# refresh-bio/kmer-db

Hardware: AMD Instinct MI355X
Metric: all2all k-mer pair-comparisons/sec (higher is better)
Workload: dtype u32

## Files before the change

kmer-db_amd/csrc/a2a_blocks.hip:

```cpp
#include "device_common.h"
#include "engine_internal.h"

#include "prim.h"

#include <algorithm>
#include <chrono>
#include <cmath>
#include <cstdio>
#include <cstdlib>
#include <cstring>

enum : uint32_t {
    KCTR_CHUNKS = 0,
    KCTR_POOL_OVERFLOW,
    KCTR_PAIR_OVERFLOW,
    KCTR_NWIDE,
    KCTR_LIST_OVERFLOW,
    KCTR_RAW = 5,
    KCTR_RECORDS = 6,
    KCTR_RECORDS_HI = 7,
    KCTR_SLOW = 8,
    KCTR_WIDE_OVERFLOW = 9,
    KCTR_WIDE_RECORDS = 10,
    KCTR_ROWJOBS = 11,
// ... 97 lines not shown
    A.t_slot = lds; A.t_key = lds + (1u << tbits); A.tmask = (1u << tbits) - 1u;
    A.sub = wave_id % KMDB_SUBPOOLS; A.wsub = A.sub; A.stock = 0; A.next = 0; A.wstock = 0; A.wnext = 0; A.dslot = 0; A.dopen = 0;
    if (tbits == 0) return;
    for (uint32_t e = lane; e <= A.tmask; e += WAVE) { A.t_slot[e] = KEY_NONE; if (!A.direct) A.t_key[e] = KEY_NONE; }
    lds_sync();
}
template <class PV> __device__ __forceinline__ uint32_t arena_take(WaveArena& A, const PV& pv, uint32_t s, uint32_t lane) {
    if (A.stock == 0) {
        uint32_t base = 0;
        A.sub = (A.sub + 61u) % KMDB_SUBPOOLS;
        if (lane == 0) base = atomicAdd(&pool_cold(pv)->sub_cursor[A.sub * 16u], ARENA_GRAB);
        base = bcast(base, 0);
        if (base + ARENA_GRAB > pool_cold(pv)->sub_cap) {
            if (lane == 0) atomicOr(&pool_cold(pv)->counters[KCTR_POOL_OVERFLOW], 1u);
            base = pool_cold(pv)->sub_cap - ARENA_GRAB;
        }
        A.next = base; A.stock = ARENA_GRAB;
    }
    const uint32_t id = A.next * KMDB_SUBPOOLS + A.sub;
    ++A.next; --A.stock;
    if (lane == 0) pool_cold(pv)->chunk_key[id] = s;
    return id;
}
template <class PV> __device__ __forceinline__ uint32_t arena_take_wide(WaveArena& A, const PV& pv, uint32_t lane) {
    if (A.wstock == 0) {
        uint32_t base = 0;
        A.wsub = (A.wsub + 61u) % KMDB_SUBPOOLS;
        if (lane == 0) base = atomicAdd(&pool_cold(pv)->wsub_cursor[A.wsub * 16u], WIDE_GRAB);
        base = bcast(base, 0);
        if (base + WIDE_GRAB > pool_cold(pv)->wsub_cap) {
            if (lane == 0) atomicOr(&pool_cold(pv)->counters[KCTR_WIDE_OVERFLOW], 1u);
            base = pool_cold(pv)->wsub_cap - WIDE_GRAB;
        }
        A.wnext = base; A.wstock = WIDE_GRAB;
    }
    const uint32_t id = A.wnext * KMDB_SUBPOOLS + A.wsub;
    ++A.wnext; --A.wstock;
    return id;
}
template <class PV> __device__ __forceinline__ Resv arena_reserve_wide(WaveArena& A, const PV& pv, uint32_t cnt, uint32_t lane) {
    if (!A.dopen) { A.dslot = arena_take_wide(A, pv, lane) << WCH_SHIFT; A.dopen = 1; }
    const uint32_t v = A.dslot, rem = WCH_REC - (v & (WCH_REC - 1u));
    if (cnt < rem) { A.dslot = v + cnt; return Resv{v, cnt, 0u}; }
    if (cnt == rem) { A.dopen = 0; return Resv{v, cnt, 0u}; }
    const uint32_t nv = arena_take_wide(A, pv, lane) << WCH_SHIFT;
    A.dslot = nv + (cnt - rem);
    return Resv{v, rem, nv};
}
__device__ __forceinline__ Resv arena_reserve(WaveArena& A, const PoolView& pv, uint32_t ent, uint32_t s, uint32_t cnt, uint32_t lane) {
    const uint32_t e = ent & A.tmask;
    uint32_t v = A.t_slot[e];
    if (A.direct) {
        if (v == KEY_NONE) v = arena_take(A, pv, s, lane) << CH_SHIFT;
    } else {
        const uint32_t key = A.t_key[e];
        if (key != s) {
            if (key != KEY_NONE && lane == 0) pv.chunk_fill[v >> CH_SHIFT] = v & (CH_REC - 1u);
            v = arena_take(A, pv, s, lane) << CH_SHIFT;
        }
    }
    const uint32_t rem = CH_REC - (v & (CH_REC - 1u));
    Resv r{v, cnt, 0u};
    uint32_t nkey = s, nv = v + cnt;
    if (cnt >= rem) {
        if (lane == 0) pv.chunk_fill[v >> CH_SHIFT] = CH_REC;
        if (cnt == rem) { nkey = KEY_NONE; nv = KEY_NONE; }
        else {
            nv = arena_take(A, pv, s, lane) << CH_SHIFT;
            r = Resv{v, rem, nv};
            nv += cnt - rem;
        }
    }
    if (lane == 0) { A.t_slot[e] = nv; if (!A.direct) A.t_key[e] = nkey; }
    lds_sync();
    return r;
}
template <class PV> __device__ __forceinline__ void arena_finish(const WaveArena& A, const PV& pv, uint32_t lane) {
    if (A.tmask == 0) return;
    for (uint32_t e = lane; e <= A.tmask; e += WAVE) {
        const uint32_t v = A.t_slot[e];
        if (v != KEY_NONE && (A.direct || A.t_key[e] != KEY_NONE)) pool_cold(pv)->chunk_fill[v >> CH_SHIFT] = v & (CH_REC - 1u);
    }
}

template <class PV> __device__ __forceinline__ void wide_emit(WaveArena& A, const PV& pv, bool on, unsigned long long rows, unsigned long long cols, uint32_t w, uint32_t stream,
                                          uint32_t lane, unsigned long long lt_mask) {
    const uint32_t dbits = pv.pshift ? (64u - pv.pshift - 2u < 16u ? 64u - pv.pshift - 2u : 16u) : pv.dbits;
    const uint32_t dmask = (1u << dbits) - 1u;
    uint32_t j = 0;
    for (;;) {
        const unsigned long long grp = __ballot(on);
        if (!grp) break;
        const Resv r = arena_reserve_wide(A, pv, (uint32_t)__popcll(grp), lane);
        if (on) {
            const uint32_t slot = resv_slot(r, (uint32_t)__popcll(grp & lt_mask));
            if (pv.pshift) {
                pv.wrec[slot] = WideRec{rows, cols | ((unsigned long long)((w & dmask) | (j << dbits)) << pv.pshift)};
                pv.wkey[slot] = stream;
            } else {
                pv.wrec[slot] = WideRec{rows, cols};
                pv.wkey[slot] = stream | (((w & dmask) | (j << dbits)) << pv.kbits);
            }
        }
        w >>= dbits; ++j;
        on = on && w != 0;
    }
}
__device__ __forceinline__ uint32_t wide_weight(uint32_t key, uint32_t kbits, uint32_t dbits) {
    const uint32_t f = key >> kbits, dig = f & ((1u << dbits) - 1u), j = f >> dbits;
    const uint32_t sh = j * dbits;
    return sh < 32u ? dig << sh : 0u;
}
struct RowTab { uint32_t* pos; uint32_t* end; uint32_t n; };
__host__ __device__ inline size_t rowtab_bytes(uint32_t n_rows) { return ((size_t)8 * n_rows + 15) & ~(size_t)15; }
__device__ __forceinline__ void rowtab_init(RowTab& R, uint32_t* lds, uint32_t n, uint32_t lane) {
    R.pos = lds; R.end = lds + n; R.n = n;
    for (uint32_t e = lane; e < 2u * n; e += WAVE) lds[e] = 0u;
    lds_sync();
}
template <class PV> __device__ __forceinline__ void row_emit(WaveArena& A, const PV& pv, const RowTab& R, bool on, uint32_t X, unsigned long long rows, unsigned long long cols,
                                         uint32_t w, uint32_t stream, uint32_t lane, unsigned long long lt_mask) {
    const uint32_t dbits = pv.pshift ? (64u - pv.pshift - 2u < 16u ? 64u - pv.pshift - 2u : 16u) : pv.dbits;
    const uint32_t dmask = (1u << dbits) - 1u;
    uint32_t j = 0;
    for (;;) {
        const unsigned long long onm = __ballot(on);
        if (!onm) break;
        const uint32_t pX = (uint32_t)__shfl_up((int)X, 1, WAVE);
        const bool lead = on && (lane == 0u || !((onm >> (lane - 1u)) & 1ull) || pX != X);
        const unsigned long long leaders = __ballot(lead);
        uint32_t ll = lane, cnt = 0;
        if (on) {
            ll = 63u - (uint32_t)__builtin_clzll(leaders & (lt_mask | (1ull << lane)));
            const unsigned long long above = ll == 63u ? 0ull : ~((2ull << ll) - 1ull);
            const unsigned long long after = (leaders | ~onm) & above;
            cnt = (after ? (uint32_t)__builtin_ctzll(after) : 64u) - ll;
        }
        uint32_t old = 0, end = 0;
        if (lead) { end = R.end[X]; old = atomicAdd(&R.pos[X], cnt); }
        uint32_t p = (uint32_t)__shfl((int)old, (int)ll, WAVE) + (lane - ll);
        const uint32_t e = (uint32_t)__shfl((int)end, (int)ll, WAVE);
        bool ovf = on && p >= e;
        unsigned long long pend = __ballot(ovf);
        while (pend) {
            const uint32_t l0 = (uint32_t)__builtin_ctzll(pend);
            const uint32_t X0 = bcast(X, l0), e0 = bcast(e, l0);
            lds_sync();
            const uint32_t tot = R.pos[X0];
            const uint32_t over = tot - e0;
            const uint32_t nnew = (over + CH_REC - 1u) >> CH_SHIFT;
            if (lane == 0 && e0) pool_cold(pv)->chunk_fill[(e0 - 1u) >> CH_SHIFT] = CH_REC;
            const bool mine = ovf && X == X0;
            const uint32_t qv = p - e0;
            uint32_t cl = 0;
            for (uint32_t i = 0; i < nnew; ++i) {
                cl = arena_take(A, pv, pool_cold(pv)->n_states + X0, lane);
                if (lane == 0 && i + 1u < nnew) pool_cold(pv)->chunk_fill[cl] = CH_REC;
                if (mine && (qv >> CH_SHIFT) == i) p = (cl << CH_SHIFT) | (qv & (CH_REC - 1u));
            }
            if (lane == 0) { R.pos[X0] = (cl << CH_SHIFT) + (over - ((nnew - 1u) << CH_SHIFT)); R.end[X0] = (cl << CH_SHIFT) + CH_REC; }
            lds_sync();
            ovf = ovf && !mine;
            pend = __ballot(ovf);
        }
        if (on) {
            if (pv.pshift) {
                ((WideRec*)pv.rec)[p] = WideRec{rows, cols | ((unsigned long long)((w & dmask) | (j << dbits)) << pv.pshift)};
                pv.recw[p] = stream;
            } else {
                ((WideRec*)pv.rec)[p] = WideRec{rows, cols};
                pv.recw[p] = stream | (((w & dmask) | (j << dbits)) << pv.kbits);
            }
        }
        w >>= dbits; ++j;
        on = on && w != 0;
    }
}
template <class PV> __device__ __forceinline__ void rowtab_finish(const RowTab& R, const PV& pv, uint32_t lane) {
    lds_sync();
    for (uint32_t X = lane; X < R.n; X += WAVE) {
        const uint32_t e = R.end[X];
        if (e) pool_cold(pv)->chunk_fill[(e - 1u) >> CH_SHIFT] = CH_REC - (e - R.pos[X]);
    }
}
template <bool ROWS, class PV>
__device__ __forceinline__ void rec_emit(WaveArena& A, const PV& pv, const RowTab& R, bool on, uint32_t X, unsigned long long rows, unsigned long long cols,
                                         uint32_t w, uint32_t stream, uint32_t lane, unsigned long long lt_mask) {
    if constexpr (ROWS) row_emit(A, pv, R, on, X, rows, cols, w, stream, lane, lt_mask);
    else wide_emit(A, pv, on, rows, cols, w, stream, lane, lt_mask);
}
__device__ __forceinline__ void rec_store_diag(const PoolView& pv, uint32_t slot, unsigned long long rows, uint32_t w) {
    const uint32_t ch = slot >> CH_SHIFT, r = slot & (CH_REC - 1u);
    ((unsigned long long*)(pv.rec + ((size_t)ch << (CH_SHIFT + 4))))[r] = rows;
    pv.recw[slot] = w;
}

__global__ void fill_u32_kernel(uint32_t* __restrict__ p, uint32_t n, uint32_t v) {
    const uint32_t i = blockIdx.x * blockDim.x + threadIdx.x;
    if (i < n) p[i] = v;
}
__global__ void iota_u32_kernel(uint32_t* __restrict__ p, uint32_t n) {
    const uint32_t i = blockIdx.x * blockDim.x + threadIdx.x;
    if (i < n) p[i] = i;
}

struct K0Params {
    const uint2* k0in;
    const uint32_t* bitrel;
    const uint64_t* blkbase;
    const uint64_t* bits;
    const uint32_t* perm;
    uint32_t P;
    uint32_t short_ids;
    BlockMap bm;
    unsigned long long* p0_mask;
    uint32_t* p0_info;
    uint32_t* pair_ofs;
    uint16_t* pair_blk;
    unsigned long long* pair_mask;
    uint32_t* pair_cursor;
    uint32_t n_regions, region_cap, spill_cap;
    uint32_t* counters;
};

constexpr int K0_RELW = 8;
constexpr int K0_SINGLE_PASS = 1;
template <bool LONG>
__global__ __launch_bounds__(256) void k0_decode_kernel(const K0Params q) {
    const uint32_t t = blockIdx.x * blockDim.x + threadIdx.x;
    const uint32_t lane = threadIdx.x & 63u;
    uint32_t i = 0;
    bool live;
    if (q.perm) {
        live = t < q.P;
        if (live) i = q.perm[t];
    } else {
        __shared__ uint32_t bins[64];
        __shared__ uint16_t order[256];
        if (threadIdx.x < 64) bins[threadIdx.x] = 0;
        __syncthreads();
        const uint2 kt = t < q.P ? q.k0in[t] : make_uint2(0u, 0u);
        const uint32_t tl = kmdb_k0_l(kt), tbits = kmdb_k0_bits(kt);
        uint32_t key = 0;
        if (t < q.P && tl > 1 && !kmdb_long_node(tl, tbits, q.short_ids)) {
            key = 1u + (tbits - (tl - 1u));
            key = key > 63u ? 63u : key;
        }
        atomicAdd(&bins[63u - key], 1u);
        __syncthreads();
        if (threadIdx.x < 64) {
            const uint32_t c = bins[threadIdx.x];
            bins[threadIdx.x] = wave_incl_scan(c, threadIdx.x) - c;
        }
        __syncthreads();
        order[atomicAdd(&bins[63u - key], 1u)] = (uint16_t)threadIdx.x;
        __syncthreads();
        i = blockIdx.x * blockDim.x + order[threadIdx.x];
        live = i < q.P;
    }
    const BlockMap bm = q.bm;
    const uint2 km = live ? q.k0in[i] : make_uint2(0u, 0u);
    const uint32_t l = kmdb_k0_l(km), last = kmdb_k0_last(km), nbits = kmdb_k0_bits(km);
    if (!q.perm && kmdb_long_node(l, nbits, q.short_ids)) live = false;
    using Cursor = RunCursor32<LONG ? 16 : 6, LONG>;
    uint32_t npairs = 0, blk0 = 0, need = 0, span = 0, bit0 = 0;
    unsigned long long mask0 = 0, m1 = 0, m2 = 0;
    bool second_pass = false, from_words = false;
    uint64_t pos = 0;
    unsigned long long rel_w[K0_RELW];
    uint32_t rel_i[K0_RELW], rel_n = 0;
#pragma unroll
    for (int e = 0; e < K0_RELW; ++e) { rel_w[e] = 0; rel_i[e] = 0; }
    auto rel_push = [&](uint32_t idx, unsigned long long w) {
#pragma unroll
        for (int e = 0; e < K0_RELW; ++e) if (rel_n == (uint32_t)e) { rel_w[e] = w; rel_i[e] = idx; }
        ++rel_n;
    };
    auto rel_blocks = [&](bool write, uint32_t id0, uint32_t o) -> uint32_t {
        const unsigned long long wm = bm.width == 64 ? ~0ull : (1ull << bm.width) - 1ull;
        uint32_t curblk = 0xFFFFFFFFu, cnt = 0;
        unsigned long long cacc = 0;
        auto flushb = [&]() {
// ... 152 lines not shown
__device__ __forceinline__ TrConst tr_const(uint32_t lane) {
    TrConst c;
    const uint32_t m[5] = {0x0000FFFFu, 0x00FF00FFu, 0x0F0F0F0Fu, 0x33333333u, 0x55555555u};
#pragma unroll
    for (int k = 0; k < 5; ++k) {
        const uint32_t s = 16u >> k;
        const bool up = (lane & s) != 0;
        c.amt[k] = up ? s : 32u - s;
        c.msk[k] = up ? m[k] : ~m[k];
    }
    return c;
}
__device__ __forceinline__ uint32_t tr_fetch(uint32_t v, int k, bool up16) {
    if (k == 0) {
        const auto a = __builtin_amdgcn_permlane16_swap(v, v, false, false);
        return up16 ? a[0] : a[1];
    }
    if (k == 1) return (uint32_t)__builtin_amdgcn_update_dpp((int)v, (int)v, 0x128, 0xF, 0xF, false);
    if (k == 2) {
        const int a = __builtin_amdgcn_update_dpp((int)v, (int)v, 0x104, 0xF, 0x5, false);
        return (uint32_t)__builtin_amdgcn_update_dpp(a, (int)v, 0x114, 0xF, 0xA, false);
    }
    if (k == 3) return (uint32_t)__builtin_amdgcn_update_dpp((int)v, (int)v, 0x4E, 0xF, 0xF, false);
    return (uint32_t)__builtin_amdgcn_update_dpp((int)v, (int)v, 0xB1, 0xF, 0xF, false);
}
__device__ __forceinline__ unsigned long long transpose64(unsigned long long x, const TrConst& c) {
    uint32_t lo = (uint32_t)x, hi = (uint32_t)(x >> 32);
    {
        const auto r = __builtin_amdgcn_permlane32_swap(lo, hi, false, false);
        lo = r[0]; hi = r[1];
    }
    const bool up16 = c.msk[0] == 0x0000FFFFu;
#pragma unroll
    for (int k = 0; k < 5; ++k) {
        const uint32_t pl = tr_fetch(lo, k, up16), ph = tr_fetch(hi, k, up16);
        const uint32_t rl = __builtin_amdgcn_alignbit(pl, pl, c.amt[k]), rh = __builtin_amdgcn_alignbit(ph, ph, c.amt[k]);
        asm("v_bfi_b32 %0, %1, %2, %0" : "+v"(lo) : "v"(c.msk[k]), "v"(rl));
        asm("v_bfi_b32 %0, %1, %2, %0" : "+v"(hi) : "v"(c.msk[k]), "v"(rh));
    }
    return ((unsigned long long)hi << 32) | lo;
}

typedef int k2_v4i __attribute__((ext_vector_type(4)));
typedef int k2_v16i __attribute__((ext_vector_type(16)));

constexpr uint32_t BNONE = 0x7FFFu;
struct NSum { unsigned long long m0, m1; uint32_t bw; };

__device__ __forceinline__ NSum nsum_make(uint32_t b0, unsigned long long m0, uint32_t b1, unsigned long long m1, bool wide) {
    return NSum{m0, m1, b0 | (b1 << 15) | ((wide ? 1u : 0u) << 30)};
}
__device__ __forceinline__ NSum nsum_merge(const NSum& T, const NSum& S) {
    const uint32_t Tb0 = T.bw & 0x7FFFu, Tb1 = (T.bw >> 15) & 0x7FFFu, Sb0 = S.bw & 0x7FFFu, Sb1 = (S.bw >> 15) & 0x7FFFu;
    bool wide = (((T.bw | S.bw) >> 30) & 1u) != 0;
    if (Tb0 == BNONE) return S;
    if (Sb0 == BNONE) return T;
    if (Sb0 == Tb0) return nsum_make(Sb0, S.m0 | T.m0, Sb1, S.m1, wide || Tb1 != BNONE);
    if (Tb1 == BNONE) return nsum_make(Tb0, T.m0, Sb0, S.m0, wide || Sb1 != BNONE);
    if (Tb1 == Sb0) return nsum_make(Tb0, T.m0, Sb0, T.m1 | S.m0, wide || Sb1 != BNONE);
    return nsum_make(Tb0, T.m0, Tb1, T.m1, true);
}
__device__ __forceinline__ NSum nsum_shfl(const NSum& s, int src) {
    return NSum{shfl64(s.m0, src), shfl64(s.m1, src), (uint32_t)__shfl((int)s.bw, src, WAVE)};
}
__device__ __forceinline__ NSum nsum_shfl_up(const NSum& s, int d) {
    return NSum{shfl_up64(s.m0, d), shfl_up64(s.m1, d), (uint32_t)__shfl_up((int)s.bw, d, WAVE)};
}

struct NParams {
    const uint32_t* nl;
    const int32_t* parent;
    const uint32_t* w;
    const uint16_t* dflag;
    const uint32_t* seg_anc;
    const uint32_t* seg_anc_n;
    const unsigned long long* p0_mask;
    const uint32_t* p0_info;
    const uint32_t* pair_ofs;
    const uint16_t* pair_blk;
    const unsigned long long* pair_mask;
    ulonglong2* fn_mask;
    uint32_t* fn_blk;
    unsigned long long* widebits;
    uint32_t P, nseg_nodes, n_segs, chain_cap;
    uint32_t emit_lo, emit_hi;
    uint32_t tbits, n_keys;
    uint32_t all_wide;
    PoolView pool;
    uint32_t* M;
    uint32_t N, bwidth;
    unsigned char* touched;
    uint32_t* direct_ctr;
    unsigned long long* dmask;
    uint32_t* dwx;
    uint32_t* slice_cnt;
    uint32_t dbg;
};
constexpr int K1N_WAVES = 4;
__host__ __device__ inline size_t k1n_wave_bytes(uint32_t chain_cap, uint32_t tbits, uint32_t n_states, uint32_t n_rows) {
    return (((size_t)chain_cap * 20 + 15) & ~(size_t)15) + arena_table_bytes(tbits, n_states) + rowtab_bytes(n_rows);
}

template <int MODE, int MINW, bool ROWS>
__global__ __launch_bounds__(WAVE * K1N_WAVES) __attribute__((amdgpu_waves_per_eu(MINW, 8))) void k1n_kernel(const NParams q) {
    constexpr bool DIRECT = MODE == 1, FLAT = MODE == 2;
    extern __shared__ __attribute__((aligned(16))) unsigned char lds_raw[];
    __shared__ unsigned long long lut_ff[DIRECT ? 256 : 1], lut_01[DIRECT ? 256 : 1];
    __shared__ __attribute__((aligned(16))) unsigned char wbuf[DIRECT ? K1N_WAVES : 1][64];
    const uint32_t lane = lane_id();
    const uint32_t wave = threadIdx.x >> 6;
    const uint32_t seg = blockIdx.x * (blockDim.x >> 6) + wave;
    if (DIRECT) {
        for (uint32_t b = threadIdx.x; b < 256u; b += blockDim.x) {
            unsigned long long v = 0;
#pragma unroll
            for (int i = 0; i < 8; ++i) v |= ((b >> i) & 1u) ? 0xFFull << (8 * i) : 0ull;
            lut_ff[b] = v;
            lut_01[b] = v & 0x0101010101010101ull;
        }
        __syncthreads();
    }
    if (seg >= q.n_segs) return;
    const uint32_t n_rows = ROWS ? q.n_keys : 0u;
    unsigned char* wbase = lds_raw + k1n_wave_bytes(q.chain_cap, q.tbits, q.n_keys, n_rows) * wave;
    uint32_t* table = (uint32_t*)wbase;
    ulonglong2* chain_m = (ulonglong2*)(wbase + arena_table_bytes(q.tbits, q.n_keys));
    uint32_t* chain_b = (uint32_t*)(chain_m + q.chain_cap);
    const unsigned long long lt_mask = (1ull << lane) - 1ull;
    RowTab RT{nullptr, nullptr, 0u};
    if constexpr (ROWS) rowtab_init(RT, (uint32_t*)(wbase + (((size_t)q.chain_cap * 20 + 15) & ~(size_t)15) + arena_table_bytes(q.tbits, q.n_keys)), n_rows, lane);
    PoolRef pv{};
    pv.k = &((KARG(NParams))__builtin_amdgcn_kernarg_segment_ptr())->pool;
    pv.kbits = q.pool.kbits; pv.dbits = q.pool.dbits; pv.pshift = q.pool.pshift;
    if constexpr (ROWS) { pv.rec = q.pool.rec; pv.recw = q.pool.recw; } else { pv.wkey = q.pool.wkey; pv.wrec = q.pool.wrec; }
    const uint32_t first = seg * q.nseg_nodes;
    const uint32_t end = (q.P - first) < q.nseg_nodes ? q.P : first + q.nseg_nodes;

    auto locals = [&](uint32_t info, unsigned long long m0, uint32_t e1blk, unsigned long long e1mask) -> NSum {
        const uint32_t np = info >> 16;
        if (np == 0) return nsum_make(BNONE, 0ull, BNONE, 0ull, false);
        if (np == 1) return nsum_make(info & 0xFFFFu, m0, BNONE, 0ull, false);
        return nsum_make(info & 0xFFFFu, m0, e1blk, e1mask, np > 2);
    };

    {
        KARG(NParams) qr = kernarg_reread<NParams>();
        const uint32_t d = qr->seg_anc_n[seg];
        NSum carry = nsum_make(BNONE, 0ull, BNONE, 0ull, false);
        for (uint32_t cb = 0; cb < d; cb += WAVE) {
            const uint32_t k = cb + lane;
            const bool on = k < d;
            NSum S = nsum_make(BNONE, 0ull, BNONE, 0ull, false);
            if (on) {
                const uint32_t node = qr->seg_anc[(size_t)seg * q.chain_cap + k];
                const uint32_t info = q.p0_info[node];
                uint32_t e1b = BNONE; unsigned long long e1m = 0;
                if ((info >> 16) > 1u) { const uint32_t po = q.pair_ofs[node]; e1b = q.pair_blk[po]; e1m = q.pair_mask[po]; }
                S = locals(info, q.p0_mask[node], e1b, e1m);
            }
            if (lane == 0) S = nsum_merge(carry, S);
#pragma unroll
            for (int s = 1; s < WAVE; s <<= 1) {
                const NSum o = nsum_shfl_up(S, s);
                if (lane >= (uint32_t)s) S = nsum_merge(o, S);
            }
            if (on) { chain_m[k] = make_ulonglong2(S.m0, S.m1); chain_b[k] = S.bw; }
            carry = nsum_shfl(S, WAVE - 1);
        }
        lds_sync();
    }

    uint32_t nx_nl = 0, nx_w = 0, nx_info = 0, nx_df = 0, nx_e1b = BNONE, nx_po = 0;
    int32_t nx_par = -1;
    unsigned long long nx_m0 = 0, nx_e1m = 0;
    uint32_t n2_nl = 0, n2_w = 0, n2_info = 0, n2_df = 0x7FFFu, n2_po = 0;
    int32_t n2_par = -1;
    unsigned long long n2_m0 = 0;
    auto fetch2 = [&](uint32_t b0) {
        const uint32_t ii = b0 + lane;
        const bool v = ii < end;
        n2_nl = v ? q.nl[ii] : 0u;
        n2_w = v ? q.w[ii] : 0u;
        n2_par = v ? q.parent[ii] : -1;
        n2_df = v ? q.dflag[ii] : 0x7FFFu;
        n2_info = v ? q.p0_info[ii] : 0u;
        n2_m0 = v ? q.p0_mask[ii] : 0ull;
        n2_po = v ? q.pair_ofs[ii] : 0u;
    };
    auto advance = [&]() {
        nx_nl = n2_nl; nx_w = n2_w; nx_par = n2_par; nx_df = n2_df; nx_info = n2_info; nx_m0 = n2_m0; nx_po = n2_po;
        nx_e1b = BNONE; nx_e1m = 0;
        if ((nx_info >> 16) > 1u) { nx_e1b = q.pair_blk[nx_po]; nx_e1m = q.pair_mask[nx_po]; }
    };
    fetch2(first); advance();
    if (first + WAVE < end) fetch2(first + WAVE); else { n2_nl = 0; n2_w = 0; n2_par = -1; n2_df = 0x7FFFu; n2_info = 0; n2_m0 = 0; n2_po = 0; }
    WaveArena A;
    arena_init(A, table, MODE != 0 ? 0u : q.tbits, q.n_keys, seg, lane);
    k2_v16i c00 = {}, c10 = {}, c11 = {};
    uint32_t curX = BNONE, n_direct = 0;
    uint32_t flat_n = 0;
    auto dflush = [&]() {
        const uint32_t half = lane >> 5, l31 = lane & 31u;
        const uint32_t rb = curX * q.bwidth;
        uint32_t* const Mb = q.M + (tri64((uint64_t)rb) + rb);
        const uint32_t lim = q.N - rb;
#pragma unroll
        for (int r = 0; r < 16; ++r) {
            const uint32_t row0 = (uint32_t)((r & 3) + 8 * (r >> 2)) + 4u * half, row1 = row0 + 32u;
            const uint32_t o0 = rb * row0 + row0 * (row0 - 1u) / 2u + l31, o1 = rb * row1 + row1 * (row1 - 1u) / 2u + l31;
            const uint32_t v00 = (uint32_t)c00[r], v10 = (uint32_t)c10[r], v11 = (uint32_t)c11[r];
            if (v00 && l31 < row0 && row0 < lim) atomicAdd(Mb + o0, v00);
            if (v10 && row1 < lim) atomicAdd(Mb + o1, v10);
            if (v11 && l31 < row0 && row1 < lim) atomicAdd(Mb + o1 + 32u, v11);
            c00[r] = 0; c10[r] = 0; c11[r] = 0;
        }
        if (lane == 0 && q.touched) q.touched[tri32(curX) + curX] = 1;
    };
    for (uint32_t base = first; base < end; base += WAVE) {
        const uint32_t idx = base + lane;
        const bool valid = idx < end;
        const uint32_t nl = nx_nl, w = nx_w, info = nx_info, df = nx_df, e1b = nx_e1b;
        const int32_t par = nx_par;
        const unsigned long long m0 = nx_m0, e1m = nx_e1m;
        if (base + WAVE < end) {
            advance();
            if (base + 2 * WAVE < end) fetch2(base + 2 * WAVE); else { n2_nl = 0; n2_w = 0; n2_par = -1; n2_df = 0x7FFFu; n2_info = 0; n2_m0 = 0; n2_po = 0; }
        }
        const uint32_t dep = df & 0x7FFFu;
        NSum S = locals(info, m0, e1b, e1m);
        if (valid && par >= 0 && par < (int32_t)base) {
            const ulonglong2 cm = chain_m[dep - 2u];
            S = nsum_merge(NSum{cm.x, cm.y, chain_b[dep - 2u]}, S);
        }
        int pl = (valid && par >= (int32_t)base) ? (int)(par - (int32_t)base) : -1;
        while (__ballot(pl >= 0)) {
            const int src = pl >= 0 ? pl : (int)lane;
            const NSum o = nsum_shfl(S, src);
            if (pl >= 0) S = nsum_merge(o, S);
            const int npl = __shfl(pl, src, WAVE);
            pl = pl >= 0 ? npl : -1;
        }
        const bool wide = valid && ((S.bw >> 30) & 1u);
        const uint32_t w0 = S.bw & 0x7FFFu, w1 = (S.bw >> 15) & 0x7FFFu;
        const unsigned long long F0 = S.m0, F1 = w1 != BNONE ? S.m1 : 0ull;
        {
            const unsigned long long wb = __ballot(wide);
            if (lane == 0) q.widebits[base >> 6] = wb;
        }
        if (__ballot(wide)) {
            const int pl0 = (valid && par >= (int32_t)base) ? (int)(par - (int32_t)base) : (int)lane;
            NSum Pp = nsum_shfl(S, pl0);
            if (valid && par >= 0 && par < (int32_t)base) { const ulonglong2 cm = chain_m[dep - 2u]; Pp = NSum{cm.x, cm.y, chain_b[dep - 2u]}; }
            if (wide && par >= 0 && !((Pp.bw >> 30) & 1u)) {
                const uint32_t pb0 = Pp.bw & 0x7FFFu, pb1 = (Pp.bw >> 15) & 0x7FFFu;
                q.fn_mask[idx] = make_ulonglong2(Pp.m0, pb1 != BNONE ? Pp.m1 : 0ull);
                q.fn_blk[idx] = (pb0 == BNONE ? 0xFFFFu : pb0) | ((pb1 == BNONE ? 0xFFFFu : pb1) << 16);
            }
        }
        const bool act = valid && !wide && w != 0 && nl >= 2u && w0 != BNONE && idx >= q.emit_lo && idx < q.emit_hi;
        auto first_block_records = [&]() {
            bool d0 = act && __popcll(F0) >= 2;
            if (FLAT) {
                const bool dd = d0 && w < 128u;
                const unsigned long long bm = __ballot(dd);
                if (dd) {
                    const uint32_t slot = first + flat_n + (uint32_t)__popcll(bm & lt_mask);
                    q.dmask[slot] = F0; q.dwx[slot] = w | (w0 << 8);
                }
                flat_n += (uint32_t)__popcll(bm);
                d0 = d0 && !dd;
            }
            if (DIRECT) {
                const bool dd = d0 && w < 128u;
                const unsigned long long pend = __ballot(dd);
                if (pend) {
                    if (curX == BNONE) curX = bcast(w0, (uint32_t)__builtin_ctzll(pend));
                    const bool mine = dd && w0 == curX;
                    n_direct += (uint32_t)__popcll(__ballot(mine));
                    if (!(q.dbg & 2u)) {
                    const TrConst trc = tr_const(lane);
                    const unsigned long long Rt = transpose64(mine ? F0 : 0ull, trc);
                    unsigned long long ra0, ra1;
                    {
                        const auto a = __builtin_amdgcn_permlane32_swap((uint32_t)Rt, (uint32_t)Rt, false, false);
                        const auto b = __builtin_amdgcn_permlane32_swap((uint32_t)(Rt >> 32), (uint32_t)(Rt >> 32), false, false);
                        ra0 = ((unsigned long long)b[0] << 32) | a[0];
                        ra1 = ((unsigned long long)b[1] << 32) | a[1];
                    }
                    wbuf[wave][lane] = (unsigned char)(mine ? w : 0u);
                    lds_sync();
                    const uint32_t half = lane >> 5;
                    auto spread = [&](unsigned long long word, uint32_t shift, const unsigned long long* lut) -> k2_v4i {
                        const uint32_t f = (uint32_t)(word >> shift) & 0xFFFFu;
                        k2_v4i r;
                        const unsigned long long lo = lut[f & 0xFFu], hi = lut[f >> 8];
                        r[0] = (int)(uint32_t)lo; r[1] = (int)(uint32_t)(lo >> 32); r[2] = (int)(uint32_t)hi; r[3] = (int)(uint32_t)(hi >> 32);
                        return r;
                    };
    #pragma unroll 1
                    for (uint32_t kh = 0; kh < 2; ++kh) {
                        const uint32_t shift = 32u * kh + 16u * half;
                        k2_v4i a0 = spread(ra0, shift, lut_ff), a1 = spread(ra1, shift, lut_ff);
                        const k2_v4i b0 = spread(ra0, shift, lut_01), b1 = spread(ra1, shift, lut_01);
                        const k2_v4i wv = *(const k2_v4i*)(wbuf[wave] + shift);
                        a0 &= wv; a1 &= wv;
                        c00 = __builtin_amdgcn_mfma_i32_32x32x32_i8(a0, b0, c00, 0, 0, 0);
                        c10 = __builtin_amdgcn_mfma_i32_32x32x32_i8(a1, b0, c10, 0, 0, 0);
                        c11 = __builtin_amdgcn_mfma_i32_32x32x32_i8(a1, b1, c11, 0, 0, 0);
                    }
                    lds_sync();
                    }
                    d0 = d0 && !mine;
                }
            }
            if (MODE == 0 && !q.all_wide) {
                unsigned long long pend = __ballot(d0);
                while (pend) {
                    const uint32_t X0 = bcast(w0, (uint32_t)__builtin_ctzll(pend));
                    const bool mine = d0 && w0 == X0;
                    const unsigned long long bc = __ballot(mine);
                    const Resv r = arena_reserve(A, q.pool, X0, tri32(X0) + X0, (uint32_t)__popcll(bc), lane);
                    if (mine) rec_store_diag(q.pool, resv_slot(r, (uint32_t)__popcll(bc & lt_mask)), F0, w);
                    pend &= ~bc;
                }
            } else {
                rec_emit<ROWS>(A, pv, RT, d0, w0, F0, F0, w, tri32(w0) + w0, lane, lt_mask);
            }
        };
        if (!DIRECT) first_block_records();
        {
            const bool act2 = act && F1 != 0;
            if (__ballot(act2)) {
                rec_emit<ROWS>(A, pv, RT, act2, w1, F1, F0, w, tri32(w1) + w0, lane, lt_mask);
                rec_emit<ROWS>(A, pv, RT, act2 && __popcll(F1) >= 2, w1, F1, F1, w, tri32(w1) + w1, lane, lt_mask);
            }
        }
        if (base + WAVE < end) {
            uint32_t m = dep;
#pragma unroll
            for (int s = 1; s < WAVE; s <<= 1) {
                const uint32_t o = (uint32_t)__shfl_down((int)m, s, WAVE);
                if (lane + (uint32_t)s < (uint32_t)WAVE) m = o < m ? o : m;
            }
            uint32_t later = (uint32_t)__shfl_down((int)m, 1, WAVE);
            if (lane == (uint32_t)WAVE - 1u) later = 0xFFFFFFFFu;
            if (valid && dep < later) { chain_m[dep - 1u] = make_ulonglong2(S.m0, S.m1); chain_b[dep - 1u] = S.bw; }
            lds_sync();
        }
        if (DIRECT) first_block_records();
    }
    if (DIRECT && curX != BNONE && !(q.dbg & 1u)) dflush();
    KARG(NParams) qe = kernarg_reread<NParams>();
    if (DIRECT && lane == 0 && n_direct) atomicAdd(&qe->direct_ctr[(seg % KMDB_SUBPOOLS) * 16u], n_direct);
    if (FLAT && lane == 0) { qe->slice_cnt[seg] = flat_n; if (flat_n) atomicAdd(&qe->direct_ctr[(seg % KMDB_SUBPOOLS) * 16u], flat_n); }
    if constexpr (MODE == 0) arena_finish(A, q.pool, lane);
    if constexpr (ROWS) rowtab_finish(RT, pv, lane);
}

constexpr uint32_t K2D_SLICES = 2;
struct DParams {
    const unsigned long long* dmask;
    const uint32_t* dwx;
    const uint32_t* slice_cnt;
    uint32_t n_segs, nseg_nodes, slices;
    uint32_t* M;
    uint32_t N, bwidth;
    unsigned char* touched;
};
__global__ __launch_bounds__(256) __attribute__((amdgpu_waves_per_eu(4, 8))) void k2d_kernel(const DParams q) {
    __shared__ unsigned long long lut_ff[256], lut_01[256];
    __shared__ __attribute__((aligned(16))) unsigned char wbuf[4][64];
    {
        unsigned long long v = 0;
#pragma unroll
        for (int i = 0; i < 8; ++i) v |= ((threadIdx.x >> i) & 1u) ? 0xFFull << (8 * i) : 0ull;
        lut_ff[threadIdx.x] = v;
        lut_01[threadIdx.x] = v & 0x0101010101010101ull;
        __syncthreads();
    }
    const uint32_t lane = threadIdx.x & 63u, wave = threadIdx.x >> 6;
    const uint32_t half = lane >> 5, l31 = lane & 31u;
    const uint32_t s0 = (blockIdx.x * 4u + wave) * q.slices;
    if (s0 >= q.n_segs) return;
    const uint32_t s1 = s0 + q.slices < q.n_segs ? s0 + q.slices : q.n_segs;
    const TrConst trc = tr_const(lane);
    auto spread = [&](unsigned long long word, uint32_t shift, const unsigned long long* lut) -> k2_v4i {
        const uint32_t f = (uint32_t)(word >> shift) & 0xFFFFu;
        k2_v4i r;
        const unsigned long long lo = lut[f & 0xFFu], hi = lut[f >> 8];
        r[0] = (int)(uint32_t)lo; r[1] = (int)(uint32_t)(lo >> 32); r[2] = (int)(uint32_t)hi; r[3] = (int)(uint32_t)(hi >> 32);
        return r;
    };
    uint32_t s = s0, n = q.slice_cnt[s0], b = 0;
    auto skip_empty = [&]() { while (b >= n && s + 1u < s1) { ++s; n = q.slice_cnt[s]; b = 0; } };
    skip_empty();
    unsigned long long nm = 0; uint32_t nwx = 0;
    auto fetch = [&]() {
        nm = 0; nwx = 0;
        if (b + lane < n) { const size_t i = (size_t)s * q.nseg_nodes + b + lane; nm = q.dmask[i]; nwx = q.dwx[i]; }
    };
    if (b < n) fetch();
    unsigned long long m = 0, pend = 0;
    uint32_t wx = 0;
    auto next_step = [&]() -> bool {
        if (b >= n) return false;
        m = nm; wx = nwx;
        b += WAVE;
        skip_empty();
        if (b < n) fetch();
        pend = __ballot(m != 0ull);
        return true;
    };
    for (;;) {
        while (!pend && next_step()) {}
        if (!pend) break;
        const uint32_t X0 = bcast(wx >> 8, (uint32_t)__builtin_ctzll(pend));
        k2_v16i c00 = {}, c10 = {}, c11 = {};
        for (;;) {
            const bool mine = ((pend >> lane) & 1ull) && (wx >> 8) == X0;
            const unsigned long long bm = __ballot(mine);
            if (!bm) break;
            pend &= ~bm;
            const unsigned long long Rt = transpose64(mine ? m : 0ull, trc);
            unsigned long long ra0, ra1;
            {
                const auto a = __builtin_amdgcn_permlane32_swap((uint32_t)Rt, (uint32_t)Rt, false, false);
                const auto c = __builtin_amdgcn_permlane32_swap((uint32_t)(Rt >> 32), (uint32_t)(Rt >> 32), false, false);
                ra0 = ((unsigned long long)c[0] << 32) | a[0];
                ra1 = ((unsigned long long)c[1] << 32) | a[1];
            }
            wbuf[wave][lane] = (unsigned char)(mine ? (wx & 0xFFu) : 0u);
            lds_sync();
#pragma unroll 1
            for (uint32_t kh = 0; kh < 2; ++kh) {
                const uint32_t shift = 32u * kh + 16u * half;
                k2_v4i a0 = spread(ra0, shift, lut_ff), a1 = spread(ra1, shift, lut_ff);
                const k2_v4i b0 = spread(ra0, shift, lut_01), b1 = spread(ra1, shift, lut_01);
                const k2_v4i wv = *(const k2_v4i*)(wbuf[wave] + shift);
                a0 &= wv; a1 &= wv;
                c00 = __builtin_amdgcn_mfma_i32_32x32x32_i8(a0, b0, c00, 0, 0, 0);
                c10 = __builtin_amdgcn_mfma_i32_32x32x32_i8(a1, b0, c10, 0, 0, 0);
                c11 = __builtin_amdgcn_mfma_i32_32x32x32_i8(a1, b1, c11, 0, 0, 0);
            }
            lds_sync();
            if (pend || !next_step()) break;
        }
        const uint32_t rb = X0 * q.bwidth;
        uint32_t* const Mb = q.M + (tri64((uint64_t)rb) + rb);
        const uint32_t lim = q.N - rb;
        uint32_t h4 = 4u * half, lc = l31;
        asm volatile("" : "+v"(h4), "+v"(lc));
#pragma unroll
        for (int r = 0; r < 16; ++r) {
            const uint32_t row0 = (uint32_t)((r & 3) + 8 * (r >> 2)) + h4, row1 = row0 + 32u;
            const uint32_t o0 = rb * row0 + row0 * (row0 - 1u) / 2u + lc, o1 = rb * row1 + row1 * (row1 - 1u) / 2u + lc;
            const uint32_t v00 = (uint32_t)c00[r], v10 = (uint32_t)c10[r], v11 = (uint32_t)c11[r];
            if (v00 && lc < row0 && row0 < lim) atomicAdd(Mb + o0, v00);
            if (v10 && row1 < lim) atomicAdd(Mb + o1, v10);
            if (v11 && lc < row0 && row1 < lim) atomicAdd(Mb + o1 + 32u, v11);
        }
        if (lane == 0 && q.touched) q.touched[tri32(X0) + X0] = 1;
    }
}

__global__ void wide_count_kernel(const unsigned long long* __restrict__ bits, uint32_t n_words, uint32_t* __restrict__ cnt) {
    const uint32_t i = blockIdx.x * blockDim.x + threadIdx.x;
    if (i < n_words) cnt[i] = (uint32_t)__popcll(bits[i]);
    else if (i == n_words) cnt[i] = 0;
}
__global__ void wide_expand_kernel(const unsigned long long* __restrict__ bits, const uint32_t* __restrict__ base, uint32_t n_words,
                                   uint32_t* __restrict__ widx, uint32_t cap, uint32_t* __restrict__ counters) {
    const uint32_t i = blockIdx.x * blockDim.x + threadIdx.x;
    if (i == 0) counters[KCTR_NWIDE] = base[n_words];
    if (i >= n_words) return;
    unsigned long long b = bits[i];
    uint32_t o = base[i];
    while (b) {
        const uint32_t k = (uint32_t)__builtin_ctzll(b);
        b &= b - 1;
        if (o < cap) widx[o] = i * 64u + k;
        ++o;
    }
}

constexpr uint32_t BLK_NONE = 0xFFFFu;
struct LSum { unsigned long long lm; uint32_t c, fb, lb; };
__device__ __forceinline__ LSum lsum_none() { return LSum{0ull, 0u, BLK_NONE, BLK_NONE}; }
__device__ __forceinline__ LSum lsum_merge(const LSum& A, const LSum& B) {
    if (B.c == 0u) return A;
    if (A.c == 0u) return B;
    const bool seam = A.lb == B.fb;
    return LSum{(B.c == 1u && seam) ? (A.lm | B.lm) : B.lm, A.c + B.c - (seam ? 1u : 0u), A.fb, B.lb};
}
__device__ __forceinline__ LSum lsum_shfl(const LSum& s, int src) {
    return LSum{shfl64(s.lm, src), (uint32_t)__shfl((int)s.c, src, WAVE), (uint32_t)__shfl((int)s.fb, src, WAVE), (uint32_t)__shfl((int)s.lb, src, WAVE)};
}
__device__ __forceinline__ LSum lsum_shfl_up(const LSum& s, int d) {
    return LSum{shfl_up64(s.lm, d), (uint32_t)__shfl_up((int)s.c, d, WAVE), (uint32_t)__shfl_up((int)s.fb, d, WAVE), (uint32_t)__shfl_up((int)s.lb, d, WAVE)};
}
__device__ __forceinline__ LSum lsum_of_fn(uint32_t fb, const ulonglong2& fm) {
    const uint32_t b0 = fb & 0xFFFFu, b1 = fb >> 16;
    if (b0 == BLK_NONE) return lsum_none();
    if (b1 == BLK_NONE) return LSum{fm.x, 1u, b0, b0};
    return LSum{fm.y, 2u, b0, b1};
}

struct L2View {
    uint32_t on, min_blocks;
    uint32_t node_cap, W;
    uint32_t ent_cap;
    uint32_t* cursors;
    unsigned long long* bitmap;
    uint32_t* ent_g;
    uint16_t* ent_blk;
    unsigned long long* ent_mask;
    uint32_t* node_w;
};
struct WParams {
    const uint32_t* widx;
    uint32_t n_wide;
    const uint32_t* nl;
    const int32_t* parent;
    const uint32_t* w;
    const uint16_t* dflag;
    const unsigned long long* widebits;
    const uint32_t* wide_base;
    const unsigned long long* p0_mask;
    const uint32_t* p0_info;
    const uint32_t* pair_ofs;
    const uint16_t* pair_blk;
    const unsigned long long* pair_mask;
    const ulonglong2* fn_mask;
    const uint32_t* fn_blk;
    const uint32_t* seg_anc;
    const uint32_t* seg_anc_n;
    uint32_t run_nodes;
    uint32_t n_runs, n_waves;
    uint32_t* run_ctr;
    uint32_t chain_cap, arena_cap, e_cap;
    uint32_t n_rows;
    uint32_t emit_lo, emit_hi;
    PoolView pool;
    L2View l2;
};
constexpr int K1W_WAVES = 2;
constexpr int K1W_MINW_FEW = 5;

constexpr uint32_t L2_MIN_BLOCKS = 24;
constexpr uint32_t L2_NODE_GRAB = 16, L2_ENT_GRAB = 1024, L2_SUB = 16;
constexpr uint32_t K1W_QCAP = 64;
constexpr uint32_t K1W_HEAVY = 11;
constexpr uint32_t K1W_OXCAP = 96;
constexpr uint32_t K1W_CTRS = 16;
constexpr uint32_t K1W_ARENA_MIN = 256;
enum : uint32_t { WB_NONE = 0, WB_FN = 1, WB_LANE = 2, WB_CHAIN = 3 };
struct K1WLds {
    unsigned long long* ent_mask;
    unsigned long long* e_mask;
    unsigned long long* ch_last;
    unsigned long long* own_m0;
    unsigned long long* own_desc;
    uint32_t* ch_node;
    unsigned long long* ox_mask;
    uint32_t* own_po;
// ... 290 lines not shown
            const uint32_t slen = len - pre;
            L.own_m0[lane] = m0; L.own_po[lane] = po;
            {
                const uint32_t nx = np > 1u ? np - 1u : 0u;
                const uint32_t xincl = wave_incl_scan(nx, lane);
                const uint32_t x0 = xincl - nx;
                const bool fits = nx && xincl <= K1W_OXCAP;
                if (fits) for (uint32_t t = 0; t < nx; ++t) { L.ox_blk[x0 + t] = qb->pair_blk[po + t]; L.ox_mask[x0 + t] = qb->pair_mask[po + t]; }
                L.own_desc[lane] = (unsigned long long)(b0 & 0xFFFFu) | ((unsigned long long)(link & 0xFFFFu) << 16) | ((unsigned long long)(fits ? x0 : 0xFFFFu) << 32) |
                                   ((unsigned long long)(np & 0x3FFFu) << 48) | ((unsigned long long)base << 62);
            }
            lds_sync();
            const bool need = valid && (act || lane == nv - 1u);
            uint32_t fin = 0, last_start = 0;
            while (fin < nv) {
                const uint32_t c = (lane >= fin && need) ? slen : 0u;
                const uint32_t incl = wave_incl_scan(c, lane);
                const unsigned long long over = __ballot(incl > qb->arena_cap);
                uint32_t hi = over ? (uint32_t)__builtin_ctzll(over) : (uint32_t)WAVE;
                if (hi <= fin) { if (lane == 0) atomicOr(&pool_cold(pv)->counters[KCTR_LIST_OVERFLOW], 1u); hi = fin + 1u; }
                const bool on = need && lane >= fin && lane < hi && incl <= qb->arena_cap;
                const uint32_t start = incl - c;
                if (on) {
                    uint32_t pos = start + slen, cur = 0xFFFFFFFFu;
                    unsigned long long curm = 0;
                    auto rflush = [&]() { if (cur != 0xFFFFFFFFu) { --pos; L.ent_blk[pos] = (uint16_t)cur; L.ent_mask[pos] = curm; } };
                    auto rpush = [&](uint32_t blk, unsigned long long mask) {
                        if (blk == cur) curm |= mask;
                        else { rflush(); cur = blk; curm = mask; }
                    };
                    uint32_t y = lane;
                    for (;;) {
                        const unsigned long long dsc = L.own_desc[y];
                        const unsigned long long ym0 = L.own_m0[y];
                        const uint32_t ynp = (uint32_t)(dsc >> 48) & 0x3FFFu, yb = (uint32_t)(dsc >> 62), ylink = (uint32_t)(dsc >> 16) & 0xFFFFu;
                        if (ynp > 1u) {
                            const uint32_t yox = (uint32_t)(dsc >> 32) & 0xFFFFu;
                            const uint32_t ynx = ynp - 1u;
                            if (yox != 0xFFFFu) for (uint32_t t = ynx; t-- > 0u;) rpush(L.ox_blk[yox + t], L.ox_mask[yox + t]);
                            else {
                                const uint32_t ypo = L.own_po[y];
                                KARG(WParams) qp = kernarg_reread<WParams>();
                                for (uint32_t t = ynx; t-- > 0u;) rpush(qp->pair_blk[ypo + t], qp->pair_mask[ypo + t]);
                            }
                        }
                        if (ynp) rpush((uint32_t)dsc & 0xFFFFu, ym0);
                        if (yb == WB_LANE) { y = ylink; continue; }
                        if (yb == WB_FN) {
                            if ((tfnb >> 16) != BLK_NONE) rpush(tfnb >> 16, tfny);
                            if ((tfnb & 0xFFFFu) != BLK_NONE) rpush(tfnb & 0xFFFFu, tfnx);
                        } else if (yb == WB_CHAIN) {
                            const uint32_t cs = ylink;
                            const uint32_t cl = L.ch_len[cs];
                            if (cl) rpush(L.e_blk[cl - 1u], L.ch_last[cs]);
                        }
                        break;
                    }
                    rflush();
                }
                L.st_start[lane] = (uint16_t)start; L.st_pre[lane] = (uint16_t)pre;
                if (lane == nv - 1u && on) last_start = start;
                lds_sync();
                emit(on && act, len, wv);
                fin = hi;
            }
            {
                uint32_t mdep = dep;
#pragma unroll
                for (int sft = 1; sft < WAVE; sft <<= 1) {
                    const uint32_t o = (uint32_t)__shfl_down((int)mdep, sft, WAVE);
                    if (lane + (uint32_t)sft < (uint32_t)WAVE) mdep = o < mdep ? o : mdep;
                }
                uint32_t later = (uint32_t)__shfl_down((int)mdep, 1, WAVE);
                if (lane == (uint32_t)WAVE - 1u) later = 0xFFFFFFFFu;
                if (valid && dep < later && dep - 1u < qb->chain_cap) { L.ch_node[dep - 1u] = node; L.ch_len[dep - 1u] = (uint16_t)len; L.ch_last[dep - 1u] = S.lm; }
                const uint32_t ll = bcast(slen, nv - 1u), ls = bcast(last_start, nv - 1u), lp = bcast(pre, nv - 1u);
                for (uint32_t e = lane; e < ll; e += WAVE) { L.e_blk[lp + e] = L.ent_blk[ls + e]; L.e_mask[lp + e] = L.ent_mask[ls + e]; }
                lds_sync();
            }
        }
    }
    arena_finish(A, pv, lane);
    if constexpr (ROWS) rowtab_finish(RT, pv, lane);
    if (lane == 0 && n_miss) atomicAdd(&pool_cold(pv)->counters[KCTR_SLOW], n_miss);
    if constexpr (L2) if (lane == 0 && l2_nodes) atomicAdd(&pool_cold(pv)->counters[KCTR_L2_NODES], l2_nodes);
}

struct K2Item {
    uint32_t X, Y, count;
    const uint32_t* ids;
    const uint32_t* fills;
    const WideRec* srec;
    const uint32_t* skey;
    uint32_t kbits, dbits;
    uint32_t pshift;
    uint32_t rect_cols;
    uint32_t n_rec;
    const unsigned char* rec;
    const uint32_t* recw;
};
constexpr uint32_t CH_STEPS = CH_REC / 64u;
template <bool SORTED>
__device__ __forceinline__ void k2_fetch(const K2Item& it, bool diag, uint32_t st, uint32_t lane, bool weighted, unsigned long long& R,
                                         unsigned long long& Cc, uint32_t& W) {
    R = 0; Cc = 0; W = 0;
    if (st >= it.count) return;
    if (SORTED) {
        const uint32_t p = st * 64u + lane;
        if (p < it.n_rec) {
            const WideRec r = it.srec[p];
            R = r.rows; Cc = r.cols;
            if (it.pshift) {
                const uint32_t f = (uint32_t)(r.cols >> it.pshift), pd = 64u - it.pshift - 2u < 16u ? 64u - it.pshift - 2u : 16u;
                const uint32_t sh = (f >> pd) * pd;
                Cc = r.cols & ((1ull << it.pshift) - 1ull);
                W = sh < 32u ? (f & ((1u << pd) - 1u)) << sh : 0u;
            } else
            W = weighted ? wide_weight(it.skey[p], it.kbits, it.dbits) : 1u;
        }
    } else {
        const uint32_t ci = st / CH_STEPS, j = (st % CH_STEPS) * 64u + lane;
        if (j < it.fills[ci]) {
            const uint32_t id = it.ids[ci];
            const unsigned char* base = it.rec + ((size_t)id << (CH_SHIFT + 4));
            if (diag) { R = ((const unsigned long long*)base)[j]; Cc = R; }
            else { const ulonglong2 rc = ((const ulonglong2*)base)[j]; R = rc.x; Cc = rc.y; }
            W = weighted ? it.recw[((size_t)id << CH_SHIFT) + j] : 1u;
        }
    }
}


template <bool DIAG, bool SORTED>
__device__ __forceinline__ uint32_t k2_apply_mfma(const K2Item& it, uint32_t digit, uint32_t* acc,
                                                  unsigned char (*wbuf)[64], const unsigned long long* lut_ff, const unsigned long long* lut_01) {
    const uint32_t lane = threadIdx.x & 63u, wave = threadIdx.x >> 6;
    const uint32_t half = lane >> 5, l31 = lane & 31u;
    k2_v16i c00 = {}, c01 = {}, c10 = {}, c11 = {};
    auto spread = [&](unsigned long long word, uint32_t shift, const unsigned long long* lut) -> k2_v4i {
        const uint32_t f = (uint32_t)(word >> shift) & 0xFFFFu;
        k2_v4i r;
        const unsigned long long lo = lut[f & 0xFFu], hi = lut[f >> 8];
        r[0] = (int)(uint32_t)lo; r[1] = (int)(uint32_t)(lo >> 32); r[2] = (int)(uint32_t)hi; r[3] = (int)(uint32_t)(hi >> 32);
        return r;
    };
    unsigned long long nR = 0, nC = 0;
    uint32_t nW = 0, wor = 0;
    const TrConst trc = tr_const(lane);
    auto next_step = [&](uint32_t st) -> uint32_t {
        if (!SORTED) while (st < it.count && (st % CH_STEPS) * 64u >= it.fills[st / CH_STEPS]) st += 4;
        return st;
    };
    uint32_t cur = next_step(wave);
    k2_fetch<SORTED>(it, DIAG, cur, lane, true, nR, nC, nW);
    while (cur < it.count) {
        const unsigned long long R = nR, C = nC;
        const uint32_t W = nW;
        cur = next_step(cur + 4);
        k2_fetch<SORTED>(it, DIAG, cur, lane, true, nR, nC, nW);
        wor |= W;
        const unsigned long long Ct = transpose64(C, trc);
        const unsigned long long Rt = DIAG ? Ct : transpose64(R, trc);
        auto halves = [&](unsigned long long w, unsigned long long& w0, unsigned long long& w1) {
            const auto a = __builtin_amdgcn_permlane32_swap((uint32_t)w, (uint32_t)w, false, false);
            const auto b = __builtin_amdgcn_permlane32_swap((uint32_t)(w >> 32), (uint32_t)(w >> 32), false, false);
            w0 = ((unsigned long long)b[0] << 32) | a[0];
// ... 242 lines not shown
        }
        const uint32_t sh = 7u * digit;
#pragma unroll
        for (int r = 0; r < 16; ++r) {
            const uint32_t row0 = (uint32_t)((r & 3) + 8 * (r >> 2)) + 4u * half;
            const uint32_t v00 = (uint32_t)c00[r] << sh, v01 = (uint32_t)c01[r] << sh, v10 = (uint32_t)c10[r] << sh, v11 = (uint32_t)c11[r] << sh;
            if (v00 && (!diag || l31 < row0)) atomicAdd(&acc[row0 * 64 + l31], v00);
            if (v01 && (!diag || 32u + l31 < row0)) atomicAdd(&acc[row0 * 64 + 32u + l31], v01);
            if (v10 && (!diag || l31 < 32u + row0)) atomicAdd(&acc[(32u + row0) * 64 + l31], v10);
            if (v11 && (!diag || l31 < row0)) atomicAdd(&acc[(32u + row0) * 64 + 32u + l31], v11);
        }
#pragma unroll
        for (int d = 32; d >= 1; d >>= 1) wor |= (uint32_t)__shfl_xor((int)wor, d, WAVE);
        if (lane == 0 && wor) atomicOr(&wor_sh, wor);
        __syncthreads();
        if (digit == 4u || (wor_sh >> (7u * (digit + 1u))) == 0) break;
        __syncthreads();
    }
    if (threadIdx.x == 0 && touched) touched[t] = 1;
    for (uint32_t k = threadIdx.x; k < 64 * 64; k += 64 * L2_WAVES) {
        const uint32_t v = acc[k];
        if (!v) continue;
        const uint64_t row = (uint64_t)X * bwidth + (k >> 6), col = (uint64_t)Y * bwidth + (k & 63u);
        if (row < N && col < row) atomicAdd(&M[tri64(row) + col], v);
    }
}

constexpr uint32_t K2_WIN = 32;
constexpr int K2A_MIN_WAVES = 3;
__global__ __launch_bounds__(256) __attribute__((amdgpu_waves_per_eu(K2A_MIN_WAVES, 8))) void k2_apply_kernel(const unsigned char* __restrict__ rec, const uint32_t* __restrict__ recw,
                                                       const uint32_t* __restrict__ sorted_key, const uint32_t* __restrict__ sorted_id,
                                                       const uint32_t* __restrict__ chunk_fill, uint32_t n_states, const uint32_t* __restrict__ n_chunks_ptr,
                                                       uint32_t* __restrict__ M, uint32_t N, uint32_t bwidth, uint32_t win, unsigned char* __restrict__ touched) {
    __shared__ uint32_t acc[64 * 64];
    __shared__ __attribute__((aligned(16))) unsigned char wbuf[4][64];
    __shared__ unsigned long long lut_ff[256], lut_01[256];
    __shared__ uint32_t s_key[K2_WIN], s_id[K2_WIN], s_fill[K2_WIN];
    __shared__ uint32_t wor_sh;
    if (threadIdx.x < win) {
        const uint32_t j = blockIdx.x * win + threadIdx.x;
        const uint32_t key = j < *n_chunks_ptr ? sorted_key[j] : n_states;
        const uint32_t id = key < n_states ? sorted_id[j] : 0u;
        s_key[threadIdx.x] = key; s_id[threadIdx.x] = id; s_fill[threadIdx.x] = key < n_states ? chunk_fill[id] : 0u;
    }
    {
        unsigned long long v = 0;
#pragma unroll
        for (int i = 0; i < 8; ++i) v |= ((threadIdx.x >> i) & 1u) ? 0xFFull << (8 * i) : 0ull;
        lut_ff[threadIdx.x] = v;
        lut_01[threadIdx.x] = v & 0x0101010101010101ull;
    }
    __syncthreads();
    uint32_t a = 0;
    while (a < win && s_key[a] < n_states) {
        const uint32_t key = s_key[a];
        uint32_t b = a + 1;
        while (b < win && s_key[b] == key) ++b;
        K2Item it;
        {
            const uint32_t bucket = key;
            uint32_t X = (uint32_t)((__fsqrt_rn(8.0f * (float)bucket + 1.0f) - 1.0f) * 0.5f);
            while (tri32(X) > bucket) --X;
            while (tri32(X + 1u) <= bucket) ++X;
            it.X = X; it.Y = bucket - tri32(X);
            it.count = (b - a) * CH_STEPS; it.ids = s_id + a; it.fills = s_fill + a; it.srec = nullptr; it.n_rec = 0; it.rec = rec; it.recw = recw; it.rect_cols = 0; it.pshift = 0;
        }
        k2_run<false>(it, acc, &wor_sh, wbuf, lut_ff, lut_01, M, N, bwidth, touched);
        a = b;
    }
}

__global__ void count_chunks_kernel(const uint32_t* __restrict__ sorted_key, uint32_t pool_cap, uint32_t n_states, uint32_t* __restrict__ counters) {
    uint32_t lo = 0, hi = pool_cap;
    while (lo < hi) { const uint32_t mid = (lo + hi) >> 1; if (sorted_key[mid] < n_states) lo = mid + 1; else hi = mid; }
    counters[KCTR_CHUNKS] = lo;
}
__global__ void pool_used_kernel(const uint32_t* __restrict__ sub_cursor, const uint32_t* __restrict__ direct_ctr, uint32_t* __restrict__ counters) {
    uint32_t mx = 0, nd = 0;
    for (uint32_t p = threadIdx.x; p < KMDB_SUBPOOLS; p += 64u) { mx = max(mx, sub_cursor[p * 16u]); nd += direct_ctr[p * 16u]; }
#pragma unroll
    for (int d = 32; d >= 1; d >>= 1) { mx = max(mx, (uint32_t)__shfl_xor((int)mx, d, WAVE)); nd += (uint32_t)__shfl_xor((int)nd, d, WAVE); }
    if (threadIdx.x == 0) { counters[KCTR_POOL_USED] = mx * KMDB_SUBPOOLS; counters[KCTR_DIRECT] = nd; }
}
__global__ void count_raw_kernel(const uint32_t* __restrict__ wsub_cursor, uint32_t* __restrict__ counters) {
    uint32_t mx = 0;
    for (uint32_t p = 0; p < KMDB_SUBPOOLS; ++p) mx = max(mx, wsub_cursor[p * 16u]);
    counters[KCTR_RAW] = mx * KMDB_SUBPOOLS;
}

constexpr uint32_t CS_MAX_KEYS = 2048, CS_BLOCKS = 2048, CS_MAX_ROWS = 512;
constexpr uint32_t CS_BLOCKS_ONE = 3072;
__device__ __forceinline__ uint32_t stream_row(uint32_t s) {
    uint32_t X = (uint32_t)((__fsqrt_rn(8.0f * (float)s + 1.0f) - 1.0f) * 0.5f);
    while (tri32(X) > s) --X;
    while (tri32(X + 1u) <= s) ++X;
    return X;
}
struct CsRows {
    const uint32_t* row_start;
    const uint32_t* row_blk;
    const uint32_t* row_tab;
    uint32_t NB, chunk;
};
enum { CS_BY_STREAM = 0, CS_BY_ROW = 1, CS_IN_ROW = 2 };
struct CsJob { uint32_t lo, hi, n_bins, sub, tab, stride; };
__device__ __forceinline__ CsJob cs_job(int mode, uint32_t n, uint32_t n_keys, const CsRows& rows) {
    CsJob j{0u, 0u, n_keys, 0u, blockIdx.x, gridDim.x};
    if (mode != CS_IN_ROW) {
        const uint32_t vb = (gridDim.x & 7u) ? blockIdx.x : xcd_contiguous(blockIdx.x, gridDim.x);
        j.tab = vb;
        const uint32_t per_block = ((n + gridDim.x - 1u) / gridDim.x + 1023u) / 1024u * 1024u;
        const uint32_t lo = vb * per_block;
        if (lo < n) { j.lo = lo; j.hi = n - lo < per_block ? n : lo + per_block; }
        return j;
    }
    j.n_bins = 0;
    if (blockIdx.x >= rows.row_blk[rows.NB]) return j;
    uint32_t a = 0, b = rows.NB;
    while (b - a > 1u) { const uint32_t mid = (a + b) >> 1; if (rows.row_blk[mid] <= blockIdx.x) a = mid; else b = mid; }
    const uint32_t X = a, c = blockIdx.x - rows.row_blk[X];
    j.lo = rows.row_start[X] + c * rows.chunk;
    j.hi = rows.row_start[X + 1];
    if (j.hi - j.lo > rows.chunk) j.hi = j.lo + rows.chunk;
    j.n_bins = X + 1u; j.sub = tri32(X); j.tab = rows.row_tab[X] + c; j.stride = rows.row_blk[X + 1] - rows.row_blk[X];
    return j;
}
__device__ __forceinline__ uint32_t cs_bin(int mode, uint32_t key, uint32_t n_valid, uint32_t sub) {
    if (key >= n_valid) return 0xFFFFFFFFu;
    return mode == CS_BY_ROW ? stream_row(key) : key - sub;
}
__global__ void cs_rows_kernel(const uint32_t* __restrict__ O1, uint32_t NB, uint32_t chunk, uint32_t* __restrict__ row_start, uint32_t* __restrict__ row_blk,
                               uint32_t* __restrict__ row_tab) {
    for (uint32_t X = threadIdx.x; X <= NB; X += blockDim.x) row_start[X] = O1[(size_t)X * CS_BLOCKS];
    __syncthreads();
    if (threadIdx.x == 0) {
        uint32_t blk = 0, tab = 0;
        for (uint32_t X = 0; X < NB; ++X) {
            row_blk[X] = blk; row_tab[X] = tab;
            const uint32_t nch = (row_start[X + 1] - row_start[X] + chunk - 1u) / chunk;
            blk += nch; tab += nch * (X + 1u);
        }
        row_blk[NB] = blk; row_tab[NB] = tab;
    }
}
__global__ __launch_bounds__(256) void cs_hist_kernel(const uint32_t* __restrict__ wkey, uint32_t n, uint32_t n_valid, uint32_t n_keys, int mode, const CsRows rows,
                                                     uint32_t kmask, uint32_t* __restrict__ H) {
    extern __shared__ uint32_t cs_lds[];
    const CsJob job = cs_job(mode, n, n_keys, rows);
    for (uint32_t k = threadIdx.x; k < job.n_bins; k += blockDim.x) cs_lds[k] = 0;
    __syncthreads();
    for (uint32_t i0 = job.lo; i0 < job.hi; i0 += 8u * blockDim.x) {
        uint32_t kw[8];
#pragma unroll
        for (uint32_t j = 0; j < 8; ++j) {
            const uint32_t i = i0 + j * blockDim.x + threadIdx.x;
            kw[j] = i < job.hi ? wkey[i] : 0xFFFFFFFFu;
        }
#pragma unroll
        for (uint32_t j = 0; j < 8; ++j) {
            const uint32_t bin = kw[j] == 0xFFFFFFFFu ? 0xFFFFFFFFu : cs_bin(mode, kw[j] & kmask, n_valid, job.sub);
            if (bin < job.n_bins) atomicAdd(&cs_lds[bin], 1u);
        }
    }
    __syncthreads();
    for (uint32_t k = threadIdx.x; k < job.n_bins; k += blockDim.x) H[(size_t)job.tab + (size_t)k * job.stride] = cs_lds[k];
    if (mode != CS_IN_ROW && blockIdx.x == 0 && threadIdx.x == 0) H[(size_t)n_keys * gridDim.x] = 0;
}
constexpr uint32_t CS_TILE = 2048, CS_THREADS = 256;
__host__ __device__ inline size_t cs_scatter_lds(uint32_t n_keys, bool packed) { return (size_t)CS_TILE * (sizeof(WideRec) + (packed ? 4 : 8)) + (size_t)n_keys * 12 + CS_THREADS * 4 + 64; }
__global__ __launch_bounds__(CS_THREADS) void cs_scatter_kernel(const uint32_t* __restrict__ wkey, const WideRec* __restrict__ wrec, uint32_t n, uint32_t n_valid,
                                                         uint32_t n_keys, int mode, const CsRows rows, uint32_t kmask, const uint32_t* __restrict__ O,
                                                         uint32_t* __restrict__ swkey, WideRec* __restrict__ swrec, uint32_t packed) {
    extern __shared__ __attribute__((aligned(16))) unsigned char cs_raw[];
    WideRec* st_rec = (WideRec*)cs_raw;
    uint32_t* st_dst = (uint32_t*)(st_rec + CS_TILE);
    uint32_t* st_key = st_dst + CS_TILE;
    uint32_t* hist = st_key + (packed ? 0u : CS_TILE);
    uint32_t* toff = hist + n_keys;
    uint32_t* cursor = toff + n_keys;
    uint32_t* part = cursor + n_keys;
    const CsJob job = cs_job(mode, n, n_keys, rows);
    const uint32_t nb = job.n_bins, lo = job.lo, hi = job.hi;
    for (uint32_t k = threadIdx.x; k < nb; k += CS_THREADS) cursor[k] = O[(size_t)job.tab + (size_t)k * job.stride];
    constexpr uint32_t PER = CS_TILE / CS_THREADS;
    const uint32_t kper = (nb + CS_THREADS - 1u) / CS_THREADS;
    uint32_t nkw[PER];
    WideRec nrec[PER];
    auto fetch = [&](uint32_t t0) {
#pragma unroll
        for (uint32_t j = 0; j < PER; ++j) {
            const uint32_t i = t0 + j * CS_THREADS + threadIdx.x;
            nkw[j] = 0xFFFFFFFFu; nrec[j] = WideRec{0ull, 0ull};
            if (i < hi) { nkw[j] = wkey[i]; nrec[j] = wrec[i]; }
        }
    };
    if (lo < hi) fetch(lo);
    for (uint32_t t0 = lo; t0 < hi; t0 += CS_TILE) {
        for (uint32_t k = threadIdx.x; k < nb; k += CS_THREADS) hist[k] = 0;
        __syncthreads();
        uint32_t key[PER], kw[PER], rank[PER];
        WideRec rc[PER];
#pragma unroll
        for (uint32_t j = 0; j < PER; ++j) {
            kw[j] = nkw[j]; rc[j] = nrec[j];
            key[j] = cs_bin(mode, kw[j] & kmask, n_valid, job.sub);
            rank[j] = key[j] < nb ? atomicAdd(&hist[key[j]], 1u) : 0u;
        }
        if (t0 + CS_TILE < hi) fetch(t0 + CS_TILE);
        __syncthreads();
        uint32_t sum = 0;
        for (uint32_t k = threadIdx.x * kper; k < nb && k < (threadIdx.x + 1u) * kper; ++k) sum += hist[k];
        const uint32_t sincl = wave_incl_scan(sum, threadIdx.x & 63u);
        if ((threadIdx.x & 63u) == 63u) part[threadIdx.x >> 6] = sincl;
        __syncthreads();
        uint32_t run = sincl - sum;
        for (uint32_t k = 0; k < (threadIdx.x >> 6); ++k) run += part[k];
        const uint32_t tile_n = part[0] + part[1] + part[2] + part[3];
        for (uint32_t k = threadIdx.x * kper; k < nb && k < (threadIdx.x + 1u) * kper; ++k) { toff[k] = run; run += hist[k]; }
        __syncthreads();
#pragma unroll
        for (uint32_t j = 0; j < PER; ++j) {
            if (key[j] < nb) {
                const uint32_t p = toff[key[j]] + rank[j];
                st_rec[p] = rc[j];
                st_dst[p] = cursor[key[j]] + rank[j];
                if (!packed) st_key[p] = kw[j];
            }
        }
        __syncthreads();
        for (uint32_t k = threadIdx.x; k < nb; k += CS_THREADS) cursor[k] += hist[k];
        for (uint32_t p = threadIdx.x; p < tile_n; p += CS_THREADS) {
            const uint32_t d = st_dst[p];
            swrec[d] = st_rec[p];
            if (!packed) swkey[d] = st_key[p];
        }
        __syncthreads();
    }
}

constexpr uint32_t CT_THREADS = 1024, CT_SLOTS = 2048;
__device__ __forceinline__ void ct_group(uint32_t key, bool on, uint32_t* t_key, uint32_t* t_cnt, uint32_t& slot, uint32_t& rank) {
    for (uint32_t e = threadIdx.x; e < CT_SLOTS; e += CT_THREADS) { t_key[e] = 0xFFFFFFFFu; t_cnt[e] = 0u; }
    __syncthreads();
    slot = 0; rank = 0;
    if (on) {
        uint32_t h = (key * 2654435761u) >> 21;
        for (;;) {
            const uint32_t prev = atomicCAS(&t_key[h], 0xFFFFFFFFu, key);
            if (prev == 0xFFFFFFFFu || prev == key) break;
            h = (h + 1u) & (CT_SLOTS - 1u);
        }
        slot = h;
        rank = atomicAdd(&t_cnt[h], 1u);
    }
    __syncthreads();
}
__global__ __launch_bounds__(CT_THREADS) void ct_hist_kernel(const uint32_t* __restrict__ chunk_key, uint32_t n, uint32_t n_keys, uint32_t* __restrict__ hist) {
    __shared__ uint32_t t_key[CT_SLOTS], t_cnt[CT_SLOTS];
    const uint32_t i = blockIdx.x * CT_THREADS + threadIdx.x;
    const uint32_t k = i < n ? chunk_key[i] : 0xFFFFFFFFu;
    uint32_t slot, rank;
    ct_group(k, k < n_keys, t_key, t_cnt, slot, rank);
    for (uint32_t e = threadIdx.x; e < CT_SLOTS; e += CT_THREADS)
        if (t_cnt[e]) atomicAdd(&hist[t_key[e]], t_cnt[e]);
}
__global__ __launch_bounds__(CT_THREADS) void ct_scatter_kernel(const uint32_t* __restrict__ chunk_key, uint32_t n, uint32_t n_keys, uint32_t* __restrict__ cursor,
                                                               uint32_t* __restrict__ sorted_key, uint32_t* __restrict__ sorted_id) {
    __shared__ uint32_t t_key[CT_SLOTS], t_cnt[CT_SLOTS];
    const uint32_t i = blockIdx.x * CT_THREADS + threadIdx.x;
    const uint32_t k = i < n ? chunk_key[i] : 0xFFFFFFFFu;
    const bool on = k < n_keys;
    uint32_t slot, rank;
    ct_group(k, on, t_key, t_cnt, slot, rank);
    for (uint32_t e = threadIdx.x; e < CT_SLOTS; e += CT_THREADS)
        if (t_cnt[e]) t_cnt[e] = atomicAdd(&cursor[t_key[e]], t_cnt[e]);
    __syncthreads();
    if (on) {
        const uint32_t o = t_cnt[slot] + rank;
// ... 330 lines not shown
    int32_t y = on ? (int32_t)node : -1;
    while (y >= 0) {
        const uint2 km = q.k0in[y];
        const uint32_t l = kmdb_k0_l(km), last = kmdb_k0_last(km);
        if (l) {
            const uint64_t pos = q.blkbase[(uint32_t)y >> 8] + q.bitrel[y];
            uint32_t sum = 0;
            if (l > 1) { BitCursor c(q.bits, pos); for (uint32_t k = 0; k + 1 < l; ++k) sum += c.next(); }
            uint32_t id = last - sum;
            uint32_t fb[EST_NW], cb[EST_NW];
#pragma unroll
            for (int c = 0; c < EST_NW; ++c) { fb[c] = __umulhi(id, q.magics[c]); cb[c] = fb[c]; nblk[c] += 1; }
            if (l > 1) {
                BitCursor c2(q.bits, pos);
                for (uint32_t k = 0; k + 1 < l; ++k) {
                    id += c2.next();
#pragma unroll
                    for (int c = 0; c < EST_NW; ++c) { const uint32_t b = __umulhi(id, q.magics[c]); nblk[c] += b != cb[c]; cb[c] = b; }
                }
            }
#pragma unroll
            for (int c = 0; c < EST_NW; ++c) { nblk[c] -= cb[c] == lower_first[c]; lower_first[c] = fb[c]; }
        }
        y = q.parent[y];
    }
    const uint32_t lane = threadIdx.x & 63u;
#pragma unroll
    for (int c = 0; c < EST_NW; ++c) {
        const unsigned long long recs = (unsigned long long)nblk[c] * (nblk[c] + 1u) / 2u;
        unsigned long long rn = on && nblk[c] >= 1u && nblk[c] <= 2u ? 1ull : 0ull;
        unsigned long long rg = on ? recs - rn : 0ull;
        unsigned long long r2 = on && nblk[c] >= q.l2_min ? recs : 0ull;
#pragma unroll
        for (int d = 32; d >= 1; d >>= 1) { rn += shfl64(rn, (int)(lane ^ (uint32_t)d)); rg += shfl64(rg, (int)(lane ^ (uint32_t)d)); r2 += shfl64(r2, (int)(lane ^ (uint32_t)d)); }
        if (lane == 0) { if (rn) atomicAdd(&q.out[c], rn); if (rg) atomicAdd(&q.out[EST_NW + c], rg); if (r2) atomicAdd(&q.out[2 * EST_NW + 1 + c], r2); }
    }
    const unsigned long long nb = __ballot(on);
    if (lane == 0 && nb) atomicAdd(&q.out[2 * EST_NW], (unsigned long long)__popcll(nb));
}

__global__ void pair_estimate_kernel(const uint2* __restrict__ k0in, const uint32_t* __restrict__ bitrel, const uint64_t* __restrict__ blkbase,
                                     const uint64_t* __restrict__ bits, uint32_t P, uint32_t stride, BlockMap bm, unsigned long long* __restrict__ out) {
    const uint32_t t = blockIdx.x * blockDim.x + threadIdx.x;
    const uint64_t i0 = (uint64_t)t * stride + (t * 2654435761u) % stride;
    unsigned long long need = 0;
    if (i0 < P) {
        const uint2 km = k0in[i0];
        const uint32_t l = kmdb_k0_l(km), last = kmdb_k0_last(km);
        if (l > 1) {
            BitCursor c(bits, blkbase[(uint32_t)i0 >> 8] + bitrel[i0]);
            uint32_t span = 0;
            for (uint32_t k = 0; k + 1 < l; ++k) span += c.next();
            const uint32_t nb = bm.blk(last) - bm.blk(last - span);
            need = nb < l - 1u ? nb : l - 1u;
        }
    }
    const uint32_t lane = threadIdx.x & 63u;
#pragma unroll
    for (int d = 32; d >= 1; d >>= 1) need += shfl64(need, (int)(lane ^ (uint32_t)d));
    if (lane == 0 && need) atomicAdd(out, need);
}

__global__ void v1_arrays_kernel(const uint2* __restrict__ k0in, const uint32_t* __restrict__ bitrel, const uint64_t* __restrict__ blkbase,
                                 const uint32_t* __restrict__ nl, uint32_t P, uint4* __restrict__ meta, uint64_t* __restrict__ bitpos) {
    const uint32_t i = blockIdx.x * blockDim.x + threadIdx.x;
    if (i >= P) return;
    const uint2 km = k0in[i];
    const uint32_t v = nl[i];
    meta[i] = make_uint4(v, kmdb_k0_l(km), kmdb_k0_last(km), kmdb_k0_bits(km));
    bitpos[i] = blkbase[i >> 8] + bitrel[i];
}

inline uint32_t wide_digit_bits(int key_bits) { return (uint32_t)(32 - key_bits - 2); }
}

struct BlocksState {
    uint32_t NB = 0, n_states = 0;
    DevBuf<unsigned long long> p0_mask;
    DevBuf<uint32_t> p0_info;
    DevBuf<uint32_t> pair_ofs;
    DevBuf<uint16_t> pair_blk;
    DevBuf<unsigned long long> pair_mask;
    uint64_t pair_cap = 0;
    DevBuf<uint32_t> pair_cursor;
    DevBuf<ulonglong2> fn_mask;
    DevBuf<uint32_t> fn_blk;
    DevBuf<unsigned long long> widebits;
    DevBuf<uint32_t> wide_cnt;
    DevBuf<uint32_t> wide_base;
    DevBuf<uint32_t> widx;
    DevBuf<uint32_t> wrun_anc;
    DevBuf<uint32_t> wrun_anc_n;
    uint64_t wide_cap = 0;
    DevBuf<uint32_t> chunk_key;
    DevBuf<uint32_t> chunk_fill;
    DevBuf<uint32_t> sorted_key;
    DevBuf<uint32_t> sorted_id;
    DevBuf<void> sort_tmp;
    size_t sort_tmp_bytes = 0;
    int key_bits = 1;
    DevBuf<unsigned char> rec;
    DevBuf<uint32_t> recw;
    uint64_t pool_cap = 0;
    DevBuf<uint32_t> sub_cursor;
    bool dense_wide = false, dense_narrow = false;
    int k1n_mode = 2;
    DevBuf<unsigned long long> dmask;
    DevBuf<uint32_t> dwx;
    DevBuf<uint32_t> slice_cnt;
    DevBuf<uint32_t> direct_ctr;
    uint64_t last_n_direct = 0;
    DevBuf<uint32_t> wkey, swkey;
    DevBuf<WideRec> wrec, swrec;
    uint64_t wide_pool_cap = 0;
    DevBuf<uint32_t> wsub_cursor;
    DevBuf<uint32_t> run_ctr;
    bool row_mode = false;
    uint32_t rec_pshift = 0;
    uint32_t n_ckeys = 0;
    DevBuf<uint32_t> ct_hist, ct_offs, ct_cursor;
    DevBuf<void> ct_tmp;
    size_t ct_tmp_bytes = 0;
    DevBuf<uint32_t> rg_hist, rg_offs;
    DevBuf<uint32_t> row_ids;
    uint32_t rg_blocks = 0;
    DevBuf<void> rg_tmp;
    size_t rg_tmp_bytes = 0;
    DevBuf<uint32_t> rs_rows;
    DevBuf<uint32_t> rs_hist, rs_offs;
    uint64_t rs_entries = 0;
    DevBuf<void> rs_tmp;
    size_t rs_tmp_bytes = 0;
    uint64_t sorted_cap = 0;
    uint32_t last_n_rowjobs = 0, last_n_sorted = 0, last_n_k2jobs = 0, k1w_waves = 0, k1w_slots = 0;
    const void* k1w_slots_fn = nullptr;
    DevBuf<uint32_t> cs_hist, cs_offs;
    DevBuf<void> cs_tmp;
    size_t cs_tmp_bytes = 0;
    DevBuf<uint32_t> counters;
    uint32_t* h_counters = nullptr;
    bool l2_on = false;
    uint32_t l2_min_blocks = 24, l2_node_cap = 0, l2_ent_cap = 0, last_l2_nodes = 0;
    DevBuf<uint32_t> l2_cursors;
    DevBuf<unsigned long long> l2_bitmap;
    DevBuf<uint32_t> l2_rank, l2_len, l2_loff;
    DevBuf<uint32_t> l2_ent_g, l2_node_w, l2_list_w;
    DevBuf<uint16_t> l2_ent_blk;
    DevBuf<unsigned long long> l2_ent_mask, l2_list_mask;
    uint64_t est_records = 0;
    bool have_counts = false;
    uint32_t last_n_wide = 0, last_n_chunks = 0, last_n_raw = 0, last_n_slow = 0;
    uint64_t last_records = 0;
    uint32_t n_slices = 1;
    struct SliceCounts { bool valid = false; uint32_t lo = 0, hi = 0, n_wide = 0, n_chunks = 0, n_raw = 0, n_rowjobs = 0, n_sorted = 0, n_k2jobs = 0; };
    std::vector<SliceCounts> slice_counts;
    DevBuf<void> scan_tmp;
    size_t scan_tmp_bytes = 0;
    DevBuf<unsigned char> tile_touched;
    DevBuf<uint32_t> k2j_start;
    DevBuf<uint2> k2j_jobs;
    uint64_t k2j_cap = 0;

    ~BlocksState() { if (h_counters) (void)hipHostFree(h_counters); }
};
void BlocksStateDelete::operator()(BlocksState* b) const { delete b; }

namespace {

PoolView pool_view(const BlocksState& b, bool dense) {
    return PoolView{b.counters, b.chunk_key, b.chunk_fill, b.rec, b.recw, b.sub_cursor, (uint32_t)(b.pool_cap / KMDB_SUBPOOLS),
                    (uint32_t)b.pool_cap, b.wkey, b.wrec, b.wsub_cursor, (uint32_t)(b.wide_pool_cap / KMDB_SUBPOOLS), dense ? 1u : 0u,
                    (uint32_t)b.key_bits, wide_digit_bits(b.key_bits), b.row_mode ? 1u : 0u, b.n_states, b.rec_pshift};
}

struct K1nPick { void (*fn)(const NParams); const char* name; };
K1nPick k1n_pick(int mode, int minw, bool rows) {
    if (mode == 2) return rows ? K1nPick{k1n_kernel<2, 4, true>, "k1n<2, rows>"} : K1nPick{k1n_kernel<2, 4, false>, "k1n<2, no rows>"};
    if (mode == 0) return rows ? K1nPick{k1n_kernel<0, 4, true>, "k1n<0, rows>"} : K1nPick{k1n_kernel<0, 4, false>, "k1n<0, no rows>"};
    if (minw >= 4) return rows ? K1nPick{k1n_kernel<1, 4, true>, "k1n<1, 4 waves, rows>"} : K1nPick{k1n_kernel<1, 4, false>, "k1n<1, 4 waves, no rows>"};
    return rows ? K1nPick{k1n_kernel<1, 3, true>, "k1n<1, 3 waves, rows>"} : K1nPick{k1n_kernel<1, 3, false>, "k1n<1, 3 waves, no rows>"};
}
struct K1wPick { void (*fn)(const WParams); const char* name; };
K1wPick k1w_pick(bool rows, bool l2) {
    if (!rows) return K1wPick{k1w_kernel<false, false>, "k1w<no rows, no L2>"};
    return l2 ? K1wPick{k1w_kernel<true, true>, "k1w<rows, L2>"} : K1wPick{k1w_kernel<true, false>, "k1w<rows, no L2>"};
}

constexpr uint32_t K1W_MAX_WAVES = 8192;
constexpr uint32_t K1W_RUN_NODES = 256;
struct U32toU64 { __host__ __device__ unsigned long long operator()(uint32_t v) const { return v; } };
struct ValidKey { uint32_t n_states, kmask; __host__ __device__ uint32_t operator()(uint32_t k) const { return (k & kmask) < n_states ? 1u : 0u; } };

inline uint64_t pool_slot_limit(const BlocksState& b) { return b.row_mode ? (1ull << 32) - (1ull << 20) : (1ull << 31); }

int alloc_record_pool(BlocksState& b, hipStream_t st, uint64_t chunks) {
    dev_reset(b.chunk_key, b.chunk_fill, b.sorted_key, b.sorted_id, b.rec, b.recw, b.sort_tmp, b.rs_hist, b.rs_offs, b.rs_tmp);
    b.pool_cap = 0;
    chunks = (chunks + (uint64_t)KMDB_SUBPOOLS * ARENA_GRAB - 1) / ((uint64_t)KMDB_SUBPOOLS * ARENA_GRAB) * ((uint64_t)KMDB_SUBPOOLS * ARENA_GRAB);
    if (chunks >= pool_slot_limit(b) >> CH_SHIFT) return kmdb_set_error("kmdb: record pool would exceed its " + std::to_string(pool_slot_limit(b)) + " record slots");
    DEV_ALLOC(b.chunk_key, chunks);
    DEV_ALLOC(b.chunk_fill, chunks);
    DEV_ALLOC(b.sorted_key, chunks);
    DEV_ALLOC(b.sorted_id, chunks);
    DEV_ALLOC(b.rec, (chunks << CH_SHIFT) * 16);
    DEV_ALLOC(b.recw, chunks << CH_SHIFT);
    {
        rocprim::transform_iterator<uint32_t*, U32toU64, unsigned long long> it(b.chunk_fill, U32toU64());
        HIP_TRY(prim::sum(nullptr, b.sort_tmp_bytes, it, (unsigned long long*)nullptr, (int)chunks, st));
    }
    DEV_ALLOC(b.sort_tmp, std::max<size_t>(b.sort_tmp_bytes, 16));
    if (b.row_mode) {
        dev_reset(b.rg_hist, b.rg_offs, b.rg_tmp, b.row_ids);
        b.rg_blocks = (uint32_t)((chunks + RG_THREADS - 1) / RG_THREADS);
        const size_t rg_ne = (size_t)b.NB * b.rg_blocks + 1;
        DEV_ALLOC(b.rg_hist, rg_ne);
        DEV_ALLOC(b.rg_offs, rg_ne);
        DEV_ALLOC(b.row_ids, chunks);
        HIP_TRY(prim::exclusive_sum(nullptr, b.rg_tmp_bytes, b.rg_hist.get(), b.rg_offs.get(), (int)rg_ne, st));
        DEV_ALLOC(b.rg_tmp, std::max<size_t>(b.rg_tmp_bytes, 16));
        b.rs_entries = (chunks / RS_JOB_CHUNKS + b.NB + 1) * (uint64_t)b.NB + 1;
        if (b.rs_entries >= (1ull << 31)) return kmdb_set_error("kmdb: the table of the sort inside the block rows would exceed 2^31 entries");
        DEV_ALLOC(b.rs_hist, b.rs_entries);
        DEV_ALLOC(b.rs_offs, b.rs_entries);
        HIP_TRY(prim::exclusive_sum(nullptr, b.rs_tmp_bytes, b.rs_hist.get(), b.rs_offs.get(), (int)b.rs_entries, st));
        DEV_ALLOC(b.rs_tmp, std::max<size_t>(b.rs_tmp_bytes, 16));
    }
    b.pool_cap = chunks;
    return 0;
}
int alloc_wide_pool(BlocksState& b, hipStream_t st, uint64_t chunks) {
    dev_reset(b.wkey, b.wrec, b.swkey, b.swrec);
    b.wide_pool_cap = 0; b.sorted_cap = 0;
    chunks = (chunks + (uint64_t)KMDB_SUBPOOLS * WIDE_GRAB - 1) / ((uint64_t)KMDB_SUBPOOLS * WIDE_GRAB) * ((uint64_t)KMDB_SUBPOOLS * WIDE_GRAB);
    const uint64_t slots = chunks << WCH_SHIFT;
    if (slots >= pool_slot_limit(b)) return kmdb_set_error("kmdb: wide record pool would exceed its " + std::to_string(pool_slot_limit(b)) + " record slots");
    DEV_ALLOC(b.swkey, slots);
    DEV_ALLOC(b.swrec, slots);
    b.sorted_cap = slots;
    b.k2j_cap = slots / K2J_REC + b.n_states + 1;
    DEV_ALLOC(b.k2j_jobs, b.k2j_cap);
// ... 42 lines not shown
    const uint64_t pos = blkbase[i >> 8] + bitrel[i];
    uint32_t sum = 0;
    { BitCursor c(bits, pos); for (uint32_t t = 0; t + 1 < l; ++t) sum += c.next(); }
    BitCursor c(bits, pos);
    uint32_t id = last - sum, o = ck_ofs[i];
    for (uint32_t t = 0; t < l; ++t) {
        if (t % KMDB_CK_IDS == 0) { ck_id[o] = id; ck_bit[o] = c.wi * 64u + c.s; ++o; }
        if (t + 1 < l) id += c.next();
    }
}

static int ensure_v1_impl(kmdb_db* db);
int kmdb_ensure_v1_arrays(kmdb_db* db) {
    if (db->v1_ready) return 0;
    if (ensure_v1_impl(db)) {
        dev_reset(db->meta, db->bitpos, db->wprefix, db->v1_counters, db->segs, db->v1_scan_tmp, db->ck_ofs, db->ck_bit, db->ck_id);
        return 1;
    }
    db->v1_ready = true;
    return 0;
}
static int ensure_v1_impl(kmdb_db* db) {
    const uint64_t P = db->P;
    DEV_ALLOC(db->meta, std::max<uint64_t>(P, 1));
    DEV_ALLOC(db->bitpos, std::max<uint64_t>(P, 1));
    DEV_ALLOC(db->wprefix, P + 1);
    DEV_ALLOC(db->v1_counters, 8);
    HIP_TRY(hipMemset(db->v1_counters, 0, 8 * sizeof(unsigned long long)));
    if (P) hipLaunchKernelGGL(v1_arrays_kernel, dim3((unsigned)((P + 255) / 256)), dim3(256), 0, db->stream, db->k0in, db->bitrel, db->blkbase, db->nl,
                              (uint32_t)P, db->meta, db->bitpos);
    HIP_TRY(hipGetLastError());
    std::vector<Segment> segs;
    const uint64_t step = 2048;
    for (uint64_t f = 0; f < P; f += step) segs.push_back(Segment{(uint32_t)f, (uint32_t)std::min<uint64_t>(P, f + step)});
    while (segs.size() % WAVES_PER_BLOCK) segs.push_back(Segment{(uint32_t)P, (uint32_t)P});
    DEV_ALLOC(db->segs, std::max<size_t>(segs.size(), 1));
    if (!segs.empty()) HIP_TRY(hipMemcpy(db->segs, segs.data(), segs.size() * sizeof(Segment), hipMemcpyHostToDevice));
    db->n_segs = (uint32_t)segs.size();
    HIP_TRY(prim::exclusive_sum(nullptr, db->v1_scan_tmp_bytes, db->w.get(), db->wprefix.get(), (int)(P + 1)));
    DEV_ALLOC(db->v1_scan_tmp, std::max<size_t>(db->v1_scan_tmp_bytes, 16));
    {
        const uint64_t P1 = P + 1;
        DevBuf<uint32_t> cnt;
        DevBuf<void> tmp;
        size_t tb = 0;
        DEV_ALLOC(cnt, P1);
        DEV_ALLOC(db->ck_ofs, P1);
        hipLaunchKernelGGL(ck_count_kernel, dim3((unsigned)((P1 + 255) / 256)), dim3(256), 0, db->stream, db->k0in, (uint32_t)P, cnt);
        HIP_TRY(prim::exclusive_sum(nullptr, tb, cnt.get(), db->ck_ofs.get(), (int)P1, db->stream));
        DEV_ALLOC(tmp, std::max<size_t>(tb, 16));
        HIP_TRY(prim::exclusive_sum(tmp, tb, cnt.get(), db->ck_ofs.get(), (int)P1, db->stream));
        uint32_t n_ck = 0;
        HIP_TRY(hipMemcpyAsync(&n_ck, db->ck_ofs + P, 4, hipMemcpyDeviceToHost, db->stream));
        HIP_TRY(hipStreamSynchronize(db->stream));
        cnt.reset(); tmp.reset();
        DEV_ALLOC(db->ck_bit, std::max<uint64_t>(n_ck, 1));
        DEV_ALLOC(db->ck_id, std::max<uint64_t>(n_ck, 1));
        if (P) hipLaunchKernelGGL(ck_fill_kernel, dim3((unsigned)((P + 255) / 256)), dim3(256), 0, db->stream, db->k0in, db->bitrel, db->blkbase, db->bits,
                                  (uint32_t)P, db->ck_ofs, db->ck_bit, db->ck_id);
        HIP_TRY(hipGetLastError());
    }
    HIP_TRY(hipStreamSynchronize(db->stream));
    return 0;
}

int kmdb_rect_sort_apply(hipStream_t st, uint32_t* wkey, void* wrec, uint32_t nslots, uint32_t nbr, uint32_t nbc, int key_bits, uint32_t* M, uint32_t n_rows,
                         uint32_t n_cols) {
    if (!nslots) return 0;
    const uint32_t n_states = nbr * nbc, kmask = (1u << key_bits) - 1u;
    DevBuf<uint32_t> swkey, hist, offs;
    DevBuf<WideRec> swrec;
    DevBuf<void> tmp;
    DEV_ALLOC(swkey, (size_t)nslots);
    DEV_ALLOC(swrec, (size_t)nslots);
    const uint32_t* total_ptr = nullptr;
    if (n_states <= CS_MAX_KEYS) {
        const size_t ne = (size_t)n_states * CS_BLOCKS_ONE + 1;
        size_t tb = 0;
        DEV_ALLOC(hist, ne);
        DEV_ALLOC(offs, ne);
        HIP_TRY(prim::exclusive_sum(nullptr, tb, hist.get(), offs.get(), (int)ne, st));
        DEV_ALLOC(tmp, std::max<size_t>(tb, 16));
        const CsRows no_rows{};
        hipLaunchKernelGGL(cs_hist_kernel, dim3(CS_BLOCKS_ONE), dim3(256), n_states * 4, st, wkey, nslots, n_states, n_states, (int)CS_BY_STREAM, no_rows, kmask, hist);
        HIP_TRY(prim::exclusive_sum(tmp, tb, hist.get(), offs.get(), (int)ne, st));
        HIP_TRY(hipFuncSetAttribute((const void*)cs_scatter_kernel, hipFuncAttributeMaxDynamicSharedMemorySize, (int)cs_scatter_lds(n_states, false)));
        hipLaunchKernelGGL(cs_scatter_kernel, dim3(CS_BLOCKS_ONE), dim3(CS_THREADS), cs_scatter_lds(n_states, false), st, wkey, (const WideRec*)wrec, nslots, n_states, n_states,
                           (int)CS_BY_STREAM, no_rows, kmask, offs, swkey, swrec, 0u);
        total_ptr = offs + (ne - 1);
    } else {
        size_t tb = 0;
        HIP_TRY(prim::sort_pairs(nullptr, tb, wkey, swkey.get(), (WideRec*)wrec, swrec.get(), (int)nslots, 0, key_bits, st));
        DEV_ALLOC(tmp, std::max<size_t>(tb, 16));
        HIP_TRY(prim::sort_pairs(tmp, tb, wkey, swkey.get(), (WideRec*)wrec, swrec.get(), (int)nslots, 0, key_bits, st));
    }
    hipLaunchKernelGGL(k2_sorted_kernel, dim3((nslots + K2S_WIN - 1) / K2S_WIN), dim3(256), 0, st, swkey, (const WideRec*)swrec, nslots, total_ptr, (const uint32_t*)nullptr,
                       n_states, (uint32_t)key_bits, wide_digit_bits(key_bits), M, n_rows, 64u, nbc, n_cols, (unsigned char*)nullptr);
    HIP_TRY(hipGetLastError());
    HIP_TRY(hipStreamSynchronize(st));
    return 0;
}

static int blocks_prepare_impl(kmdb_db* db);
int kmdb_blocks_prepare(kmdb_db* db) {
    db->blocks.reset(new BlocksState());
    if (blocks_prepare_impl(db)) { kmdb_blocks_release(db); return 1; }
    db->blocks_prepared = true;
    return 0;
}
static int blocks_prepare_impl(kmdb_db* db) {
    BlocksState& b = *db->blocks;
    const uint64_t N = db->N, P = db->P;
    db->fallback_reason.clear();
    if (N < 2 || P == 0) { db->fallback_reason = "fewer than two samples"; return 0; }
    if (!db->chain_ok) {
        db->fallback_reason = "a root path of " + std::to_string(db->max_depth) + " nodes exceeds the chain table (" + std::to_string(KMDB_CHAIN_MAX) + ")";
        return 0;
    }
    const bool verbose = getenv("KMDB_VERBOSE") != nullptr;
    auto t_mark = std::chrono::steady_clock::now();
    auto phase = [&](const char* what) {
        if (!verbose) return;
        (void)hipStreamSynchronize(db->stream);
        const auto now = std::chrono::steady_clock::now();
        fprintf(stderr, "[kmdb] prepare: %-36s %.3f s\n", what, std::chrono::duration<double>(now - t_mark).count());
        t_mark = now;
    };
    const uint32_t cands[EST_NW] = {64, 60, 56, 52, 50, 48, 44, 40, 36, 32};
    uint32_t forced = 0;
    if (const char* e = getenv("KMDB_BLOCK_WIDTH")) forced = (uint32_t)strtoul(e, nullptr, 10);
    const uint32_t stride = (uint32_t)std::max<uint64_t>(1, std::min<uint64_t>(1024, P / 65536));
    uint64_t est_n = 0, est_g = 0, est_l2 = 0;
    {
        EstParams q{};
        q.k0in = db->k0in; q.bitrel = db->bitrel; q.blkbase = db->blkbase; q.bits = db->bits; q.parent = db->parent; q.nl = db->nl; q.w = db->w;
        q.P = (uint32_t)P; q.stride = stride;
        for (int c = 0; c < EST_NW; ++c) { q.widths[c] = cands[c]; q.magics[c] = (uint32_t)((1ull << 32) / cands[c]) + 1u; }
        q.l2_min = getenv("KMDB_L2_MIN") ? std::max<uint32_t>(K1W_HEAVY, (uint32_t)atoi(getenv("KMDB_L2_MIN"))) : L2_MIN_BLOCKS;
        DevBuf<unsigned long long> d_out;
        DEV_ALLOC(d_out, 3 * EST_NW + 1);
        q.out = d_out;
        HIP_TRY(hipMemsetAsync(q.out, 0, (3 * EST_NW + 1) * 8, db->stream));
        const uint64_t nthreads = (P + stride - 1) / stride;
        hipLaunchKernelGGL(width_estimate_kernel, dim3((unsigned)((nthreads + 63) / 64)), dim3(64), 0, db->stream, q);
        HIP_TRY(hipGetLastError());
        unsigned long long h[3 * EST_NW + 1];
        HIP_TRY(hipMemcpyAsync(h, q.out, sizeof h, hipMemcpyDeviceToHost, db->stream));
        HIP_TRY(hipStreamSynchronize(db->stream));
        int best = 0;
        for (int c = 1; c < EST_NW; ++c) if (h[c] + h[EST_NW + c] < h[best] + h[EST_NW + best]) best = c;
        if (forced >= 32 && forced <= 64) {
            db->width = forced;
            best = 0;
            for (int c = 0; c < EST_NW; ++c) if (cands[c] >= forced) best = c;
        } else db->width = cands[best];
        est_n = h[best] * stride; est_g = h[EST_NW + best] * stride; est_l2 = h[2 * EST_NW + 1 + best] * stride;
        b.est_records = est_n + est_g;
        if (verbose) {
            fprintf(stderr, "[kmdb] width estimate (1 node in %u, %llu sampled):", stride, h[2 * EST_NW]);
            for (int c = 0; c < EST_NW; ++c) fprintf(stderr, " %u:%llu", cands[c], (h[c] + h[EST_NW + c]) * stride);
            fprintf(stderr, " -> width %u\n", db->width);
        }
    }
    b.NB = (uint32_t)((N + db->width - 1) / db->width);
    const uint64_t n_states = (uint64_t)b.NB * (b.NB + 1) / 2;
    if (n_states + 1 >= (1ull << 22)) { db->fallback_reason = "too many block pairs"; return 0; }
    static_assert((1ull << 22) < (uint64_t)BNONE * (BNONE + 1ull) / 2ull, "fewer than 2^22 block pairs keep the block index (< 2897) below BNONE and inside pair_blk's 16 bits");
    b.n_states = (uint32_t)n_states;
    if (k1w_wave_bytes(std::max<uint32_t>(K1W_ARENA_MIN, (b.NB + 2u + 63u) & ~63u), (b.NB + 2u + 3u) & ~3u, db->chain_cap, b.NB) > (size_t)(152u << 10)) {
        db->fallback_reason = "the lists of the wide-node kernel do not fit the LDS (" + std::to_string(b.NB) + " blocks, root paths of up to " +
                              std::to_string(db->max_depth) + " nodes)";
        return 0;
    }
    phase("block width estimate");
    DEV_ALLOC(b.p0_mask, P);
    DEV_ALLOC(b.p0_info, P);
    DEV_ALLOC(b.pair_ofs, P);
    DEV_ALLOC(b.pair_cursor, (KMDB_PAIR_REGIONS + 1) * 16);
    DEV_ALLOC(b.fn_mask, P);
    DEV_ALLOC(b.fn_blk, P);
    const uint64_t n_words = (P + 63) / 64;
    DEV_ALLOC(b.widebits, n_words);
    DEV_ALLOC(b.wide_cnt, n_words + 1);
    DEV_ALLOC(b.wide_base, n_words + 1);
    HIP_TRY(prim::exclusive_sum(nullptr, b.scan_tmp_bytes, b.wide_cnt.get(), b.wide_base.get(), (int)(n_words + 1)));
    DEV_ALLOC(b.scan_tmp, std::max<size_t>(b.scan_tmp_bytes, 16));
    DEV_ALLOC(b.counters, KCTR_COUNT);
    HIP_TRY(hipHostMalloc((void**)&b.h_counters, KCTR_COUNT * 4));
    phase("per-node arrays (hipMalloc)");
    {
        DevBuf<unsigned long long> d_need;
        DEV_ALLOC(d_need, 1);
        HIP_TRY(hipMemsetAsync(d_need, 0, 8, db->stream));
        const BlockMap bm{db->width, (uint32_t)((1ull << 32) / db->width) + 1u};
        const uint64_t nthreads = (P + stride - 1) / stride;
        hipLaunchKernelGGL(pair_estimate_kernel, dim3((unsigned)((nthreads + 63) / 64)), dim3(64), 0, db->stream, db->k0in, db->bitrel, db->blkbase, db->bits,
                           (uint32_t)P, stride, bm, d_need);
        unsigned long long h_need = 0;
        HIP_TRY(hipMemcpyAsync(&h_need, d_need, 8, hipMemcpyDeviceToHost, db->stream));
        HIP_TRY(hipStreamSynchronize(db->stream));
        d_need.reset();
        const uint64_t est_pairs = h_need * stride;
        if (verbose) fprintf(stderr, "[kmdb] extra (block, mask) pairs, sampled: %llu\n", (unsigned long long)est_pairs);
        if (alloc_pair_pool(b, std::max<uint64_t>(est_pairs * 2 + P / 4, (uint64_t)KMDB_PAIR_REGIONS * 64))) return 1;
    }
    phase("pair estimate + pair pool");
    DEV_ALLOC(b.sub_cursor, KMDB_SUBPOOLS * 16);
    DEV_ALLOC(b.wsub_cursor, KMDB_SUBPOOLS * 16);
    DEV_ALLOC(b.run_ctr, K1W_CTRS * 16);
    DEV_ALLOC(b.direct_ctr, KMDB_SUBPOOLS * 16);
    b.dense_wide = true;
    b.dense_narrow = false;
    if (const char* e = getenv("KMDB_DENSE")) b.dense_narrow = atoi(e) >= 2;
    b.k1n_mode = 2;
    if (const char* e = getenv("KMDB_K1N_MODE")) if (*e) b.k1n_mode = std::max(0, std::min(2, atoi(e)));
    if (b.k1n_mode) b.dense_narrow = true;
    if (b.k1n_mode == 2) {
        const size_t slots = (size_t)db->n_nsegs * db->nseg_nodes;
        DEV_ALLOC(b.dmask, std::max<size_t>(slots, 1));
        DEV_ALLOC(b.dwx, std::max<size_t>(slots, 1));
        DEV_ALLOC(b.slice_cnt, std::max<size_t>(db->n_nsegs, 1));
    }
    b.row_mode = b.n_states > CS_MAX_KEYS;
    if (const char* e = getenv("KMDB_ROW_MODE")) if (*e) b.row_mode = atoi(e) != 0;
    b.rec_pshift = (db->width <= 54u && !(getenv("KMDB_REC_PACKED") && getenv("KMDB_REC_PACKED")[0] == '0')) ? db->width : 0u;
    {
        const char* l2_env = getenv("KMDB_L2");
        if (b.row_mode && b.NB <= 256u && !(l2_env && l2_env[0] == '0')) {
            if (verbose) fprintf(stderr, "[kmdb] block records estimated: %llu, of them %llu from nodes the second level joins per tile instead\n",
                                 (unsigned long long)(est_n + est_g), (unsigned long long)est_l2);
            est_g -= std::min(est_g, est_l2);
        }
    }
    b.n_ckeys = b.n_states;
    {
        int key_bits = 1;
        while ((1ull << key_bits) <= (uint64_t)b.n_states + 1) ++key_bits;
        b.key_bits = key_bits;
    }
    DEV_ALLOC(b.tile_touched, (size_t)b.n_states + 1);
    DEV_ALLOC(b.ct_hist, (size_t)b.n_ckeys + 2);
    DEV_ALLOC(b.ct_offs, (size_t)b.n_ckeys + 2);
    DEV_ALLOC(b.ct_cursor, (size_t)b.n_ckeys + 2);
    HIP_TRY(prim::exclusive_sum(nullptr, b.ct_tmp_bytes, b.ct_hist.get(), b.ct_offs.get(), (int)(b.n_ckeys + 1), db->stream));
    DEV_ALLOC(b.ct_tmp, std::max<size_t>(b.ct_tmp_bytes, 16));
    {
        uint64_t slices = 1;
        const uint64_t slots = (est_n + est_g) * 3 / 2;
        const uint64_t usable = pool_slot_limit(b) / 4 * 3;
        slices = std::max<uint64_t>(slices, (slots + usable - 1) / usable);
        size_t free_b = 0, total_b = 0;
        if (hipMemGetInfo(&free_b, &total_b) == hipSuccess && free_b)
            slices = std::max<uint64_t>(slices, (slots * 44 + free_b / 2) / std::max<size_t>(free_b * 6 / 10, 1));
        if (const char* e = getenv("KMDB_SLICES")) if (*e) slices = std::max<uint64_t>(1, strtoull(e, nullptr, 10));
        b.n_slices = (uint32_t)std::min<uint64_t>(slices, 1u << 16);
        if (verbose && b.n_slices > 1) fprintf(stderr, "[kmdb] %llu block records estimated: %u slices of the pattern stream per call\n",
                                                 (unsigned long long)(est_n + est_g), b.n_slices);
        est_n = est_n / b.n_slices + 1; est_g = est_g / b.n_slices + 1;
    }
    if (const char* e = getenv("KMDB_POOL_PERCENT")) if (*e) {
        const uint64_t pct = std::max<uint64_t>(1, strtoull(e, nullptr, 10));
        est_n = est_n * pct / 100 + 1; est_g = est_g * pct / 100 + 1;
    }
    b.k1w_waves = K1W_MAX_WAVES;
    if (b.row_mode) {
        b.k1w_waves = std::min<uint32_t>(b.k1w_waves, std::max<uint32_t>(256u, std::min<uint32_t>(4096u, (1u << 21) / std::max<uint32_t>(b.NB, 1u))));
        DEV_ALLOC(b.rs_rows, (size_t)2 * (b.NB + 1));
    }
    DEV_ALLOC(b.k2j_start, (size_t)b.n_states + 2);
    if (b.k1n_mode) { est_g += est_n / 16 + 1; est_n = 0; }
    if (b.row_mode) {
        if (alloc_record_pool(b, db->stream, (est_n + est_g) * 5 / 4 / CH_REC + (uint64_t)db->n_nsegs * std::min<uint32_t>(b.NB, 48u) + (uint64_t)b.k1w_waves * (b.NB + ARENA_GRAB) + 4096)) return 1;
        if (alloc_wide_pool(b, db->stream, (est_n + est_g) * 9 / 8 / WCH_REC + 4096)) return 1;
    } else {
        if (alloc_record_pool(b, db->stream, est_n * 3 / 2 / CH_REC + (b.dense_narrow ? 0u : (uint64_t)db->n_nsegs * 8) + 4096)) return 1;
        if (alloc_wide_pool(b, db->stream, est_g * 3 / 2 / WCH_REC + (uint64_t)(K1W_MAX_WAVES + 64) * (WIDE_GRAB + 2) + (uint64_t)db->n_nsegs * (WIDE_GRAB / 2) + 1024)) return 1;
    }
    if (verbose) fprintf(stderr, "[kmdb] prepare: record pools %.2f GB\n", kmdb_blocks_device_bytes(db) / 1e9);
    phase("record pools (hipMalloc)");
    return 0;
}

void kmdb_blocks_release(kmdb_db* db) { db->blocks.reset(); }

uint64_t kmdb_blocks_device_bytes(const kmdb_db* db) {
    if (!db->blocks || !db->blocks->counters) return 0;
    const BlocksState& b = *db->blocks;
    return db->P * (8 + 4 + 4 + 16 + 4) + (b.dmask ? (uint64_t)db->n_nsegs * db->nseg_nodes * 12 : 0u) + b.pair_cap * 10 + ((b.pool_cap << CH_SHIFT) * 20) + b.pool_cap * 16 + b.wide_cap * 4 + (db->P / 64) * 16 +
           (b.wide_pool_cap << WCH_SHIFT) * (b.row_mode ? 20 : 40) + b.rs_entries * 8 + (uint64_t)b.n_ckeys * 12 +
           (uint64_t)b.NB * (b.l2_node_cap / 64u) * 12 + (uint64_t)b.l2_ent_cap * 26 + (uint64_t)b.l2_node_cap * 4;
}

namespace {

int alloc_l2(BlocksState& b, uint32_t node_cap, uint32_t ent_cap) {
    dev_reset(b.l2_cursors, b.l2_bitmap, b.l2_rank, b.l2_len, b.l2_loff, b.l2_ent_g, b.l2_node_w, b.l2_list_w, b.l2_ent_blk, b.l2_ent_mask, b.l2_list_mask);
    b.l2_node_cap = 0; b.l2_ent_cap = 0;
    node_cap = (node_cap + 64u * L2_SUB - 1u) / (64u * L2_SUB) * (64u * L2_SUB);
    ent_cap = (ent_cap + L2_ENT_GRAB * L2_SUB - 1u) / (L2_ENT_GRAB * L2_SUB) * (L2_ENT_GRAB * L2_SUB);
    const size_t W = node_cap / 64u, NB = b.NB;
    DEV_ALLOC(b.l2_cursors, 2 * L2_SUB * 16);
    DEV_ALLOC(b.l2_bitmap, NB * W);
    DEV_ALLOC(b.l2_rank, NB * W);
    DEV_ALLOC(b.l2_len, NB);
    DEV_ALLOC(b.l2_loff, NB + 2);
    DEV_ALLOC(b.l2_ent_g, (size_t)ent_cap);
    DEV_ALLOC(b.l2_ent_blk, (size_t)ent_cap);
    DEV_ALLOC(b.l2_ent_mask, (size_t)ent_cap);
    DEV_ALLOC(b.l2_list_mask, (size_t)ent_cap);
    DEV_ALLOC(b.l2_list_w, (size_t)ent_cap);
    DEV_ALLOC(b.l2_node_w, (size_t)node_cap);
    b.l2_node_cap = node_cap; b.l2_ent_cap = ent_cap;
    return 0;
}

int blocks_attempt(kmdb_db* db, uint32_t* M, uint32_t emit_lo, uint32_t emit_hi, bool decode, hipStream_t st, bool* retry) {
    BlocksState& b = *db->blocks;
    *retry = false;
    static const bool sync_debug = getenv("KMDB_SYNC_DEBUG") != nullptr;
    auto stage = [&](const char* name) -> int {
        if (!sync_debug) return 0;
        const hipError_t e = hipStreamSynchronize(st);
        fprintf(stderr, "[kmdb] stage %-14s %s\n", name, e == hipSuccess ? "ok" : hipGetErrorString(e));
        return e == hipSuccess ? 0 : kmdb_set_error(std::string("stage ") + name + ": " + hipGetErrorString(e));
    };
    const uint32_t P = (uint32_t)db->P;
    const BlockMap bm{db->width, (uint32_t)((1ull << 32) / db->width) + 1u};
    const uint32_t n_words = (P + 63) / 64;
    const uint32_t pool_cap = (uint32_t)b.pool_cap;
    const bool row_mode = b.row_mode;
    const uint32_t n_ckeys = b.n_ckeys;
    HIP_TRY(hipMemsetAsync(b.counters, 0, KCTR_COUNT * 4, st));
    if (decode) HIP_TRY(hipMemsetAsync(b.pair_cursor, 0, (KMDB_PAIR_REGIONS + 1) * 16 * 4, st));
    HIP_TRY(hipMemsetAsync(b.sub_cursor, 0, KMDB_SUBPOOLS * 16 * 4, st));
    HIP_TRY(hipMemsetAsync(b.wsub_cursor, 0, KMDB_SUBPOOLS * 16 * 4, st));
    HIP_TRY(hipMemsetAsync(b.run_ctr, 0, K1W_CTRS * 16 * 4, st));
    HIP_TRY(hipMemsetAsync(b.direct_ctr, 0, KMDB_SUBPOOLS * 16 * 4, st));
    auto with_slack = [](uint32_t v) -> uint32_t { return v + v / 8u + 1024u; };
    const uint32_t raw_launch = b.have_counts ? (uint32_t)std::min<uint64_t>(with_slack(b.last_n_raw), row_mode ? 0xFFFFFFFFull : b.wide_pool_cap) : 0u;
    if (!row_mode) {
        const uint64_t wslots = b.have_counts ? (uint64_t)raw_launch << WCH_SHIFT : b.wide_pool_cap << WCH_SHIFT;
        HIP_TRY(hipMemsetAsync(b.wkey, 0xFF, wslots * 4, st));
    }
    HIP_TRY(hipMemsetAsync(b.chunk_fill, 0, (size_t)pool_cap * 4, st));
    HIP_TRY(hipMemsetAsync(b.ct_hist, 0, ((size_t)n_ckeys + 2) * 4, st));
    hipLaunchKernelGGL(fill_u32_kernel, dim3((pool_cap + 255) / 256), dim3(256), 0, st, b.chunk_key, pool_cap, 0xFFFFFFFFu);
    if (stage("init")) return 1;
    if (decode) {
        K0Params q{};
        q.k0in = db->k0in; q.bitrel = db->bitrel; q.blkbase = db->blkbase; q.bits = db->bits; q.perm = nullptr; q.P = P; q.short_ids = db->short_max_ids; q.bm = bm;
        q.p0_mask = b.p0_mask; q.p0_info = b.p0_info; q.pair_ofs = b.pair_ofs; q.pair_blk = b.pair_blk; q.pair_mask = b.pair_mask;
        uint32_t nreg = 1;
        while (nreg < KMDB_PAIR_REGIONS && (uint64_t)nreg * 16384 < P) nreg <<= 1;
        q.pair_cursor = b.pair_cursor; q.n_regions = nreg; q.region_cap = (uint32_t)(b.pair_cap * 3 / 4 / nreg);
        q.spill_cap = (uint32_t)(b.pair_cap - (uint64_t)q.region_cap * nreg); q.counters = b.counters;
        hipLaunchKernelGGL((k0_decode_kernel<false>), dim3((P + 255) / 256), dim3(256), 0, st, q);
        if (db->n_long) {
            q.perm = db->long_nodes; q.P = db->n_long;
            hipLaunchKernelGGL((k0_decode_kernel<true>), dim3((db->n_long + 255) / 256), dim3(256), 0, st, q);
        }
        HIP_TRY(hipGetLastError());
    }
    if (stage("decode")) return 1;
    HIP_TRY(hipEventRecord(db->ev_k[0], st));
    {
        NParams q{};
        q.nl = db->nl; q.parent = db->parent; q.w = db->w; q.dflag = db->dflag; q.seg_anc = db->nseg_anc; q.seg_anc_n = db->nseg_anc_n;
        q.p0_mask = b.p0_mask; q.p0_info = b.p0_info; q.pair_ofs = b.pair_ofs; q.pair_blk = b.pair_blk; q.pair_mask = b.pair_mask;
        q.fn_mask = b.fn_mask; q.fn_blk = b.fn_blk; q.widebits = b.widebits;
        q.P = P; q.nseg_nodes = db->nseg_nodes; q.n_segs = db->n_nsegs; q.chain_cap = db->chain_cap;
        q.emit_lo = emit_lo; q.emit_hi = emit_hi; q.tbits = b.dense_narrow ? 0u : arena_table_bits(b.NB); q.n_keys = b.NB;
        q.all_wide = b.dense_narrow ? 1u : 0u;
        q.pool = pool_view(b, b.dense_narrow);
        const size_t wave_lds = k1n_wave_bytes(q.chain_cap, q.tbits, q.n_keys, row_mode ? b.NB : 0u);
        const uint32_t waves = (uint32_t)std::max<size_t>(1, std::min<size_t>(K1N_WAVES, (144u << 10) / wave_lds));
        const size_t lds = wave_lds * waves;
        q.dbg = getenv("KMDB_K1N_DBG") ? (uint32_t)atoi(getenv("KMDB_K1N_DBG")) : 0u;
        q.M = M; q.N = (uint32_t)db->N; q.bwidth = db->width; q.touched = b.tile_touched; q.direct_ctr = b.direct_ctr;
        q.dmask = b.dmask; q.dwx = b.dwx; q.slice_cnt = b.slice_cnt;
        static const int minw = getenv("KMDB_K1N_MINW") ? atoi(getenv("KMDB_K1N_MINW")) : 3;
        const K1nPick pick = k1n_pick(b.k1n_mode, minw, row_mode);
        HIP_TRY(hipFuncSetAttribute((const void*)pick.fn, hipFuncAttributeMaxDynamicSharedMemorySize, (int)lds));
        const dim3 grid((q.n_segs + waves - 1) / waves), block(WAVE * waves);
        if (!b.have_counts && getenv("KMDB_VERBOSE"))
            fprintf(stderr, "[kmdb] narrow kernel: %u slices, %zu B of LDS per wave, %u per workgroup, instantiation %s\n", q.n_segs, wave_lds, waves, pick.name);
        hipLaunchKernelGGL(pick.fn, grid, block, lds, st, q);
        HIP_TRY(hipGetLastError());
    }
    if (stage("narrow emit")) return 1;
    HIP_TRY(hipEventRecord(db->ev_k[1], st));
    hipStream_t s2 = db->stream2;
    auto group_and_apply_chunks = [&](hipStream_t cs) -> int {
        hipLaunchKernelGGL(ct_hist_kernel, dim3((pool_cap + CT_THREADS - 1) / CT_THREADS), dim3(CT_THREADS), 0, cs, b.chunk_key, pool_cap, n_ckeys, b.ct_hist);
        size_t tb = b.ct_tmp_bytes;
        HIP_TRY(prim::exclusive_sum(b.ct_tmp, tb, b.ct_hist.get(), b.ct_offs.get(), (int)(n_ckeys + 1), cs));
        HIP_TRY(hipMemcpyAsync(b.ct_cursor, b.ct_offs, ((size_t)n_ckeys + 1) * 4, hipMemcpyDeviceToDevice, cs));
        hipLaunchKernelGGL(ct_scatter_kernel, dim3((pool_cap + CT_THREADS - 1) / CT_THREADS), dim3(CT_THREADS), 0, cs, b.chunk_key, pool_cap, n_ckeys, b.ct_cursor, b.sorted_key, b.sorted_id);
        hipLaunchKernelGGL(ct_count_kernel, dim3(1), dim3(1), 0, cs, b.ct_offs, b.n_states, b.counters);
        if (cs != s2) { HIP_TRY(hipEventRecord(db->ev_side[0], cs)); HIP_TRY(hipStreamWaitEvent(s2, db->ev_side[0], 0)); }
        {
            rocprim::transform_iterator<uint32_t*, U32toU64, unsigned long long> it(b.chunk_fill, U32toU64());
            HIP_TRY(prim::sum(b.sort_tmp, b.sort_tmp_bytes, it, (unsigned long long*)(b.counters + KCTR_RECORDS), (int)pool_cap, s2));
        }
        const uint32_t win = b.n_states <= CS_MAX_KEYS ? 16u : 32u;
        uint32_t grid = (pool_cap + win - 1) / win;
        if (b.have_counts) grid = std::min(grid, (b.last_n_chunks + win - 1) / win);
        if (grid)
            hipLaunchKernelGGL(k2_apply_kernel, dim3(grid), dim3(256), 0, s2, b.rec, b.recw, b.sorted_key, b.sorted_id, b.chunk_fill, b.n_states,
                               b.ct_offs + b.n_states, M, (uint32_t)db->N, db->width, win, b.tile_touched);
        HIP_TRY(hipGetLastError());
        HIP_TRY(hipEventRecord(db->ev_side[1], s2));
        if (sync_debug) { const hipError_t e = hipStreamSynchronize(s2); fprintf(stderr, "[kmdb] stage %-14s %s\n", "chunk apply", e == hipSuccess ? "ok" : hipGetErrorString(e)); }
        return 0;
    };
    auto apply_slices = [&]() -> int {
        HIP_TRY(hipEventRecord(db->ev_side[0], st));
        HIP_TRY(hipStreamWaitEvent(s2, db->ev_side[0], 0));
        DParams d{};
        d.dmask = b.dmask; d.dwx = b.dwx; d.slice_cnt = b.slice_cnt; d.n_segs = db->n_nsegs; d.nseg_nodes = db->nseg_nodes;
        static const uint32_t sl = getenv("KMDB_K2D_SLICES") ? (uint32_t)std::max(1, atoi(getenv("KMDB_K2D_SLICES"))) : K2D_SLICES;
        d.slices = sl; d.M = M; d.N = (uint32_t)db->N; d.bwidth = db->width; d.touched = b.tile_touched;
        const uint32_t waves = (db->n_nsegs + sl - 1u) / sl;
        if (waves) hipLaunchKernelGGL(k2d_kernel, dim3((waves + 3u) / 4u), dim3(256), 0, s2, d);
        HIP_TRY(hipGetLastError());
        HIP_TRY(hipEventRecord(db->ev_side[1], s2));
        if (sync_debug) { const hipError_t e = hipStreamSynchronize(s2); fprintf(stderr, "[kmdb] stage %-14s %s\n", "slice apply", e == hipSuccess ? "ok" : hipGetErrorString(e)); }
        return 0;
    };
    static const bool k2d_early = !(getenv("KMDB_K2D_EARLY") && getenv("KMDB_K2D_EARLY")[0] == '0');
    if (b.k1n_mode == 2 && k2d_early && apply_slices()) return 1;
    if (!row_mode) {
        if (!b.dense_narrow) {
            HIP_TRY(hipEventRecord(db->ev_side[0], st));
            HIP_TRY(hipStreamWaitEvent(s2, db->ev_side[0], 0));
            if (group_and_apply_chunks(s2)) return 1;
        } else HIP_TRY(hipEventRecord(db->ev_side[1], s2));
    }
    hipLaunchKernelGGL(wide_count_kernel, dim3((n_words + 1 + 255) / 256), dim3(256), 0, st, b.widebits, n_words, b.wide_cnt);
    HIP_TRY(prim::exclusive_sum(b.scan_tmp, b.scan_tmp_bytes, b.wide_cnt.get(), b.wide_base.get(), (int)(n_words + 1), st));
    uint32_t n_wide;
    if (b.have_counts && b.wide_cap >= b.last_n_wide) n_wide = b.last_n_wide;
    else {
        HIP_TRY(hipMemcpyAsync(b.h_counters, b.wide_base + n_words, 4, hipMemcpyDeviceToHost, st));
        HIP_TRY(hipStreamSynchronize(st));
        n_wide = b.h_counters[0];
        if (n_wide > b.wide_cap) {
            dev_reset(b.widx, b.wrun_anc, b.wrun_anc_n);
            b.wide_cap = 0;
            DEV_ALLOC(b.widx, (size_t)n_wide);
            DEV_ALLOC(b.wrun_anc, ((size_t)n_wide / 64 + 1) * db->chain_cap);
            DEV_ALLOC(b.wrun_anc_n, (size_t)n_wide / 64 + 1);
            b.wide_cap = n_wide;
        }
    }
    if (!b.widx) { DEV_ALLOC(b.widx, 1); b.wide_cap = std::max<uint64_t>(b.wide_cap, 1); }
    hipLaunchKernelGGL(wide_expand_kernel, dim3((n_words + 255) / 256), dim3(256), 0, st, b.widebits, b.wide_base, n_words, b.widx,
                       (uint32_t)b.wide_cap, b.counters);
    if (b.k1n_mode == 2 && !k2d_early && apply_slices()) return 1;
    if (n_wide) {
        WParams q{};
        q.widx = b.widx; q.n_wide = n_wide; q.nl = db->nl; q.parent = db->parent; q.w = db->w; q.widebits = b.widebits;
        q.dflag = db->dflag; q.wide_base = b.wide_base;
        q.p0_mask = b.p0_mask; q.p0_info = b.p0_info; q.pair_ofs = b.pair_ofs; q.pair_blk = b.pair_blk; q.pair_mask = b.pair_mask;
        q.fn_mask = b.fn_mask; q.fn_blk = b.fn_blk; q.emit_lo = emit_lo; q.emit_hi = emit_hi; q.pool = pool_view(b, b.dense_wide);
        {
            const char* l2_env = getenv("KMDB_L2");
            const char* l2_min_env = getenv("KMDB_L2_MIN");
            b.l2_on = row_mode && b.NB <= 256u && !(l2_env && l2_env[0] == '0');
            b.l2_min_blocks = l2_min_env ? std::max<uint32_t>(K1W_HEAVY, (uint32_t)atoi(l2_min_env)) : L2_MIN_BLOCKS;
            if (b.l2_on && !b.l2_bitmap) {
                const bool tiny = getenv("KMDB_POOL_PERCENT") != nullptr;
                if (alloc_l2(b, tiny ? 1u : std::max<uint32_t>(64u * L2_SUB * 4u, n_wide / 16u), tiny ? 1u : std::max<uint32_t>(L2_ENT_GRAB * L2_SUB * 4u, n_wide / 16u * 48u))) return 1;
            }
            q.l2 = L2View{};
            if (b.l2_on) {
                q.l2.on = 1u; q.l2.min_blocks = b.l2_min_blocks; q.l2.node_cap = b.l2_node_cap; q.l2.W = b.l2_node_cap / 64u; q.l2.ent_cap = b.l2_ent_cap;
                q.l2.cursors = b.l2_cursors; q.l2.bitmap = b.l2_bitmap; q.l2.ent_g = b.l2_ent_g; q.l2.ent_blk = b.l2_ent_blk; q.l2.ent_mask = b.l2_ent_mask;
                q.l2.node_w = b.l2_node_w;
                HIP_TRY(hipMemsetAsync(b.l2_cursors, 0, 2 * L2_SUB * 16 * 4, st));
                HIP_TRY(hipMemsetAsync(b.l2_bitmap, 0, (size_t)b.NB * q.l2.W * 8, st));
                HIP_TRY(hipMemsetAsync(b.l2_ent_blk, 0xFF, (size_t)b.l2_ent_cap * 2, st));
            }
        }
        q.run_nodes = K1W_RUN_NODES;
        if (const char* e = getenv("KMDB_K1W_RUN")) q.run_nodes = std::max<uint32_t>(64u, (uint32_t)atoi(e) / 64u * 64u);
        q.n_runs = (n_wide + q.run_nodes - 1) / q.run_nodes;
        hipLaunchKernelGGL(wrun_anc_kernel, dim3((q.n_runs + 63) / 64), dim3(64), 0, st, b.widx, n_wide, q.run_nodes, db->parent, db->dflag, db->chain_cap,
                           b.wrun_anc, b.wrun_anc_n);
        q.seg_anc = b.wrun_anc; q.seg_anc_n = b.wrun_anc_n;
        
        q.chain_cap = db->chain_cap; q.e_cap = (b.NB + 2u + 3u) & ~3u; q.arena_cap = std::max<uint32_t>(K1W_ARENA_MIN, (b.NB + 2u + 63u) & ~63u);
        q.n_rows = row_mode ? b.NB : 0u;
        const size_t wave_lds = k1w_wave_bytes(q.arena_cap, q.e_cap, q.chain_cap, q.n_rows);
        const uint32_t waves = wave_lds * K1W_WAVES <= (size_t)(64u << 10) ? (uint32_t)K1W_WAVES : 1u;
        const K1wPick pick = k1w_pick(row_mode, b.l2_on);
        HIP_TRY(hipFuncSetAttribute((const void*)pick.fn, hipFuncAttributeMaxDynamicSharedMemorySize, (int)(wave_lds * waves)));
        if (!b.k1w_slots || b.k1w_slots_fn != (const void*)pick.fn) {
            int per_cu = 0, dev = 0;
            hipDeviceProp_t prop;
            b.k1w_slots = 0; b.k1w_slots_fn = (const void*)pick.fn;
            HIP_TRY(hipOccupancyMaxActiveBlocksPerMultiprocessor(&per_cu, (const void*)pick.fn, (int)(WAVE * waves), wave_lds * waves));
            HIP_TRY(hipGetDevice(&dev));
            HIP_TRY(hipGetDeviceProperties(&prop, dev));
            b.k1w_slots = (uint32_t)std::max(1, per_cu) * waves * (uint32_t)std::max(1, prop.multiProcessorCount);
        }
        q.n_waves = std::min<uint32_t>(std::min<uint32_t>(b.k1w_slots, b.k1w_waves), q.n_runs);
        q.run_ctr = b.run_ctr;
        if (const char* e = getenv("KMDB_K1W_WAVES")) q.n_waves = std::max<uint32_t>(1u, std::min<uint32_t>(std::min<uint32_t>(b.k1w_waves, q.n_runs), (uint32_t)atoi(e)));
        if (!b.have_counts && getenv("KMDB_VERBOSE"))
            fprintf(stderr, "[kmdb] wide kernel: %u wide nodes in %u runs, %u waves (%u fit the chip, %zu B of LDS per wave, %u per workgroup), instantiation %s\n", n_wide,
                    q.n_runs, q.n_waves, b.k1w_slots, wave_lds, waves, pick.name);
        hipLaunchKernelGGL(pick.fn, dim3((q.n_waves + waves - 1) / waves), dim3(WAVE * waves), wave_lds * waves, st, q);
        if (b.l2_on) {
            const uint32_t NB = b.NB, W = b.l2_node_cap / 64u;
            hipLaunchKernelGGL(l2_ranks_kernel, dim3(NB), dim3(256), 0, st, b.l2_bitmap, W, b.l2_rank, b.l2_len);
            hipLaunchKernelGGL(l2_offsets_kernel, dim3(1), dim3(64), 0, st, b.l2_len, NB, b.l2_cursors, W, b.l2_loff);
            hipLaunchKernelGGL(l2_lists_kernel, dim3((b.l2_ent_cap + 255u) / 256u), dim3(256), 0, st, b.l2_ent_g, b.l2_ent_blk, b.l2_ent_mask, b.l2_node_w,
                               b.l2_ent_cap, W, b.l2_bitmap, b.l2_rank, b.l2_loff, b.l2_list_mask, b.l2_list_w, b.l2_cursors);
            hipLaunchKernelGGL(l2_join_apply_kernel, dim3(NB * (NB + 1u) / 2u), dim3(64 * L2_WAVES), 0, st, b.l2_bitmap, b.l2_rank, b.l2_list_mask, b.l2_list_w,
                               b.l2_loff, W, NB, M, (uint32_t)db->N, db->width, b.tile_touched);
        }
    }
    HIP_TRY(hipGetLastError());
    if (stage("wide emit")) return 1;
    HIP_TRY(hipEventRecord(db->ev_k[2], st));
    const uint32_t kmask = (1u << b.key_bits) - 1u;
    uint32_t jobs_launched = 0, k2jobs_launched = 0;
    if (row_mode) {
        if (group_and_apply_chunks(st)) return 1;
        const uint32_t NB = b.NB;
        uint32_t* row_job = b.rs_rows, *row_tab = b.rs_rows + (NB + 1);
        {
            const size_t rg_ne = (size_t)NB * b.rg_blocks + 1;
            hipLaunchKernelGGL(rg_hist_kernel, dim3(b.rg_blocks), dim3(RG_THREADS), NB * 4, st, b.chunk_key, pool_cap, b.n_states, NB, b.rg_hist);
            size_t tbg = b.rg_tmp_bytes;
            HIP_TRY(prim::exclusive_sum(b.rg_tmp, tbg, b.rg_hist.get(), b.rg_offs.get(), (int)rg_ne, st));
            hipLaunchKernelGGL(rg_scatter_kernel, dim3(b.rg_blocks), dim3(RG_THREADS), NB * 4, st, b.chunk_key, pool_cap, b.n_states, NB, b.rg_offs, b.row_ids);
        }
        hipLaunchKernelGGL(rs_rows_kernel, dim3(1), dim3(1024), 0, st, b.rg_offs, b.rg_blocks, NB, row_job, row_tab, b.counters);
        const RsRows R{b.rg_offs, b.row_ids, b.rg_blocks, NB, row_job, row_tab};
        const uint32_t jobs_bound = (uint32_t)(pool_cap / RS_JOB_CHUNKS + NB + 1);
        const uint32_t jobs = b.have_counts ? std::min<uint32_t>(jobs_bound, with_slack(b.last_n_rowjobs)) : jobs_bound;
        jobs_launched = jobs;
        const size_t ne = std::min<size_t>(b.rs_entries, (size_t)jobs * NB + 1);
        HIP_TRY(hipMemsetAsync(b.rs_hist, 0, ne * 4, st));
        {
            const char* ue = getenv("KMDB_RSH_UNROLL");
            const int u = ue ? atoi(ue) : 16;
            if (u == 16) hipLaunchKernelGGL(rs_hist_kernel<16>, dim3(jobs), dim3(256), NB * 4, st, R, b.chunk_fill, b.recw, kmask, b.rs_hist);
            else if (u == 8) hipLaunchKernelGGL(rs_hist_kernel<8>, dim3(jobs), dim3(256), NB * 4, st, R, b.chunk_fill, b.recw, kmask, b.rs_hist);
            else hipLaunchKernelGGL(rs_hist_kernel<4>, dim3(jobs), dim3(256), NB * 4, st, R, b.chunk_fill, b.recw, kmask, b.rs_hist);
        }
        size_t tb = b.rs_tmp_bytes;
        HIP_TRY(prim::exclusive_sum(b.rs_tmp, tb, b.rs_hist.get(), b.rs_offs.get(), (int)ne, st));
        const uint32_t* total_ptr = b.rs_offs + (ne - 1);
        HIP_TRY(hipMemcpyAsync(b.counters + KCTR_WIDE_RECORDS, total_ptr, 4, hipMemcpyDeviceToDevice, st));
        HIP_TRY(hipFuncSetAttribute((const void*)rs_scatter_kernel, hipFuncAttributeMaxDynamicSharedMemorySize, (int)rs_scatter_lds(NB, b.rec_pshift != 0)));
        hipLaunchKernelGGL(rs_scatter_kernel, dim3((jobs + 7u) & ~7u), dim3(CS_THREADS), rs_scatter_lds(NB, b.rec_pshift != 0), st, R, b.chunk_fill, b.recw, (const WideRec*)b.rec.get(), kmask,
                           b.rs_offs, (uint32_t)b.sorted_cap, b.swkey, (WideRec*)b.swrec, b.counters, b.rec_pshift ? 1u : 0u);
        hipLaunchKernelGGL(k2j_starts_kernel, dim3((b.n_states + 1u + 255u) / 256u), dim3(256), 0, st, R, b.rs_offs, b.n_states, b.k2j_start);
        hipLaunchKernelGGL(k2j_build_kernel, dim3((b.n_states + 1023u) / 1024u), dim3(1024), 0, st, b.k2j_start, b.n_states, b.k2j_jobs, (uint32_t)b.k2j_cap, b.counters);
        k2jobs_launched = b.have_counts ? b.last_n_k2jobs : (uint32_t)b.k2j_cap;
        if (k2jobs_launched)
            hipLaunchKernelGGL(k2_jobs_kernel, dim3(k2jobs_launched), dim3(256), 0, st, b.swkey, (const WideRec*)b.swrec, b.k2j_start, b.k2j_jobs, b.counters + KCTR_K2JOBS,
                               (uint32_t)b.k2j_cap, (uint32_t)b.sorted_cap, b.rec_pshift, (uint32_t)b.key_bits, wide_digit_bits(b.key_bits), M, (uint32_t)db->N, db->width, b.tile_touched);
        HIP_TRY(hipGetLastError());
        if (stage("row sort+apply")) return 1;
    } else {
        hipLaunchKernelGGL(count_raw_kernel, dim3(1), dim3(1), 0, st, b.wsub_cursor, b.counters);
        uint32_t n_raw;
        if (b.have_counts) n_raw = raw_launch;
        else {
            HIP_TRY(hipMemcpyAsync(b.h_counters, b.counters, KCTR_COUNT * 4, hipMemcpyDeviceToHost, st));
            HIP_TRY(hipStreamSynchronize(st));
            n_raw = std::min<uint32_t>(b.h_counters[KCTR_RAW], (uint32_t)b.wide_pool_cap);
        }
        if (n_raw) {
            const uint32_t nslots = (uint32_t)((uint64_t)n_raw << WCH_SHIFT);
            const CsRows no_rows{};
            const size_t ne = (size_t)b.n_states * CS_BLOCKS_ONE + 1;
            hipLaunchKernelGGL(cs_hist_kernel, dim3(CS_BLOCKS_ONE), dim3(256), b.n_states * 4, st, b.wkey, nslots, b.n_states, b.n_states, (int)CS_BY_STREAM,
                               no_rows, kmask, b.cs_hist);
            size_t tb = b.cs_tmp_bytes;
            HIP_TRY(prim::exclusive_sum(b.cs_tmp, tb, b.cs_hist.get(), b.cs_offs.get(), (int)ne, st));
            const bool packed = b.rec_pshift != 0;
            HIP_TRY(hipFuncSetAttribute((const void*)cs_scatter_kernel, hipFuncAttributeMaxDynamicSharedMemorySize, (int)cs_scatter_lds(b.n_states, packed)));
            hipLaunchKernelGGL(cs_scatter_kernel, dim3(CS_BLOCKS_ONE), dim3(CS_THREADS), cs_scatter_lds(b.n_states, packed), st, b.wkey, (const WideRec*)b.wrec, nslots,
                               b.n_states, b.n_states, (int)CS_BY_STREAM, no_rows, kmask, b.cs_offs, b.swkey, (WideRec*)b.swrec, packed ? 1u : 0u);
            const uint32_t* total_ptr = b.cs_offs + (ne - 1);
            HIP_TRY(hipMemcpyAsync(b.counters + KCTR_WIDE_RECORDS, total_ptr, 4, hipMemcpyDeviceToDevice, st));
            if (getenv("KMDB_K2_WINDOWS") && !packed) {
                const uint32_t g2 = (nslots + K2S_WIN - 1) / K2S_WIN;
                hipLaunchKernelGGL(k2_sorted_kernel, dim3(g2), dim3(256), 0, st, b.swkey, (const WideRec*)b.swrec, nslots, total_ptr, (const uint32_t*)nullptr,
                                   b.n_states, (uint32_t)b.key_bits, wide_digit_bits(b.key_bits), M, (uint32_t)db->N, db->width, 0u, 0u, b.tile_touched);
            } else {
                hipLaunchKernelGGL(k2j_starts_flat_kernel, dim3((b.n_states + 1u + 255u) / 256u), dim3(256), 0, st, b.cs_offs, b.n_states, CS_BLOCKS_ONE, b.k2j_start);
                hipLaunchKernelGGL(k2j_build_kernel, dim3((b.n_states + 1023u) / 1024u), dim3(1024), 0, st, b.k2j_start, b.n_states, b.k2j_jobs, (uint32_t)b.k2j_cap, b.counters);
                k2jobs_launched = b.have_counts ? b.last_n_k2jobs : (uint32_t)b.k2j_cap;
                if (k2jobs_launched)
                    hipLaunchKernelGGL(k2_jobs_kernel, dim3(k2jobs_launched), dim3(256), 0, st, b.swkey, (const WideRec*)b.swrec, b.k2j_start, b.k2j_jobs, b.counters + KCTR_K2JOBS,
                                       (uint32_t)b.k2j_cap, (uint32_t)b.sorted_cap, b.rec_pshift, (uint32_t)b.key_bits, wide_digit_bits(b.key_bits), M, (uint32_t)db->N, db->width, b.tile_touched);
            }
            HIP_TRY(hipGetLastError());
        }
        if (stage("sorted apply")) return 1;
    }
    HIP_TRY(hipStreamWaitEvent(st, db->ev_side[1], 0));
    hipLaunchKernelGGL(pool_used_kernel, dim3(1), dim3(64), 0, st, b.sub_cursor, b.direct_ctr, b.counters);
    HIP_TRY(hipEventRecord(db->ev_k[3], st));
    HIP_TRY(hipMemcpyAsync(b.h_counters, b.counters, KCTR_COUNT * 4, hipMemcpyDeviceToHost, st));
    HIP_TRY(hipStreamSynchronize(st));
    const uint32_t* c = b.h_counters;
    if (c[KCTR_LIST_OVERFLOW] || c[KCTR_SLOW]) {
        db->fallback_reason = "internal: the wide-node kernel lost a list (chain miss " + std::to_string(c[KCTR_SLOW]) + ", arena overflow " + std::to_string(c[KCTR_LIST_OVERFLOW]) + ")";
        return 0;
    }
    if (c[KCTR_L2_OVERFLOW]) {
        if (getenv("KMDB_VERBOSE")) fprintf(stderr, "[kmdb] second level out of node indices or entries (%u / %u): doubling\n", b.l2_node_cap, b.l2_ent_cap);
        if (alloc_l2(b, b.l2_node_cap * 2u, b.l2_ent_cap * 2u)) return 1;
        b.have_counts = false; *retry = true;
        return 0;
    }
    if (c[KCTR_PAIR_OVERFLOW] || c[KCTR_POOL_OVERFLOW] || c[KCTR_WIDE_OVERFLOW]) {
        const bool verbose = getenv("KMDB_VERBOSE") != nullptr;
        if (c[KCTR_PAIR_OVERFLOW]) {
            if (verbose) fprintf(stderr, "[kmdb] pair pool too small (%llu entries): doubling\n", (unsigned long long)b.pair_cap);
            if (alloc_pair_pool(b, b.pair_cap * 2)) return 1;
        }
        if (c[KCTR_WIDE_OVERFLOW]) {
            const uint64_t want = b.wide_pool_cap * 2;
            if ((want << WCH_SHIFT) >= pool_slot_limit(b)) {
                if (b.n_slices >= (1u << 16)) { db->fallback_reason = "more block records than a pool can index from the nodes with many blocks in a 65536th of the patterns"; return 0; }
                b.n_slices *= 2;
                if (verbose) fprintf(stderr, "[kmdb] wide record pool at its limit: %u slices of the pattern stream per call\n", b.n_slices);
                b.have_counts = false; *retry = true;
                return 0;
            }
            if (verbose) fprintf(stderr, "[kmdb] wide record pool too small (%llu chunks): doubling\n", (unsigned long long)b.wide_pool_cap);
            if (alloc_wide_pool(b, db->stream, want)) return 1;
        }
        if (c[KCTR_POOL_OVERFLOW]) {
            uint64_t want = b.pool_cap * 2;
            if (!row_mode && !b.dense_narrow && b.n_states > (1u << ST_MAX_BITS) && (b.pool_cap << CH_SHIFT) > 8 * (b.est_records + (1u << 22))) {
                b.dense_narrow = true;
                if (verbose) fprintf(stderr, "[kmdb] record chunks of the narrow kernel are evicted nearly empty: its records go through the sort too\n");
                if (alloc_wide_pool(b, db->stream, b.wide_pool_cap + b.est_records * 5 / 4 / WCH_REC + (uint64_t)db->n_nsegs * (WIDE_GRAB + 2))) return 1;
                want = 0;
            } else if (row_mode && !b.dense_narrow && b.NB > (1u << ST_MAX_BITS) && (b.pool_cap << CH_SHIFT) > 8 * (b.est_records + (1u << 22))) {
                b.dense_narrow = true;
                if (verbose) fprintf(stderr, "[kmdb] record chunks of the narrow kernel are evicted nearly empty: its records go through the row chunks too\n");
                if (alloc_wide_pool(b, db->stream, b.wide_pool_cap + b.est_records * 5 / 4 / WCH_REC)) return 1;
                want = 0;
            } else if ((want << CH_SHIFT) >= pool_slot_limit(b)) {
                if (b.n_slices >= (1u << 16)) {
                    db->fallback_reason = "more block records than a pool can index in a 65536th of the patterns (" + std::to_string(b.n_states) + " streams, " + std::to_string(b.pool_cap) + " chunks were not enough)";
                    return 0;
                }
                b.n_slices *= 2;
                if (verbose) fprintf(stderr, "[kmdb] record pool at its limit: %u slices of the pattern stream per call\n", b.n_slices);
                b.have_counts = false; *retry = true;
                return 0;
            }
            if (want) {
                if (verbose) fprintf(stderr, "[kmdb] record pool too small (%llu chunks): %llu\n", (unsigned long long)b.pool_cap, (unsigned long long)want);
                if (alloc_record_pool(b, db->stream, want)) return 1;
            }
        }
        b.have_counts = false; *retry = true;
        return 0;
    }
    if (b.have_counts && (c[KCTR_NWIDE] != b.last_n_wide || c[KCTR_CHUNKS] != b.last_n_chunks ||
                            (row_mode ? (c[KCTR_ROWJOBS] > jobs_launched || c[KCTR_WIDE_RECORDS] != b.last_n_sorted || c[KCTR_K2JOBS] > k2jobs_launched)
                                      : (c[KCTR_RAW] > raw_launch || c[KCTR_K2JOBS] > k2jobs_launched)))) {
        if (getenv("KMDB_VERBOSE"))
            fprintf(stderr, "[kmdb] a launch was sized too small (wide nodes %u / %u, chunks %u / %u, row jobs %u / %u, sorted %u / %u, apply jobs %u / %u, raw %u / %u): the call is repeated\n",
                    c[KCTR_NWIDE], b.last_n_wide, c[KCTR_CHUNKS], b.last_n_chunks, c[KCTR_ROWJOBS], jobs_launched, c[KCTR_WIDE_RECORDS], b.last_n_sorted, c[KCTR_K2JOBS],
                    k2jobs_launched, c[KCTR_RAW], raw_launch);
        b.have_counts = false; *retry = true;
        return 0;
    }
    if ((uint64_t)c[KCTR_POOL_USED] * 100 > b.pool_cap * 85) {
        if (getenv("KMDB_VERBOSE")) fprintf(stderr, "[kmdb] record pool %u of %llu chunks in use: enlarged by a quarter\n", c[KCTR_POOL_USED], (unsigned long long)b.pool_cap);
        const uint64_t want = b.pool_cap + b.pool_cap / 4;
        if (((want + (uint64_t)KMDB_SUBPOOLS * ARENA_GRAB) << CH_SHIFT) < pool_slot_limit(b) && alloc_record_pool(b, db->stream, want)) return 1;
    }
    if (!row_mode && (uint64_t)c[KCTR_RAW] * 100 > b.wide_pool_cap * 85) {
        if (getenv("KMDB_VERBOSE")) fprintf(stderr, "[kmdb] wide record pool %u of %llu chunks in use: enlarged by a quarter\n", c[KCTR_RAW], (unsigned long long)b.wide_pool_cap);
        const uint64_t want = b.wide_pool_cap + b.wide_pool_cap / 4;
        if (((want + (uint64_t)KMDB_SUBPOOLS * WIDE_GRAB) << WCH_SHIFT) < pool_slot_limit(b) && alloc_wide_pool(b, db->stream, want)) return 1;
    }
    if (!b.have_counts && getenv("KMDB_VERBOSE"))
        fprintf(stderr, "[kmdb] record pool: %u of %llu chunks in use (busiest sub-pool x sub-pools); wide pool / sorted arrays: %llu slots\n", c[KCTR_POOL_USED],
                (unsigned long long)b.pool_cap, (unsigned long long)b.sorted_cap);
    b.last_n_wide = c[KCTR_NWIDE]; b.last_n_chunks = c[KCTR_CHUNKS]; b.last_n_raw = c[KCTR_RAW]; b.last_n_slow = c[KCTR_SLOW];
    b.last_n_rowjobs = c[KCTR_ROWJOBS]; b.last_n_sorted = c[KCTR_WIDE_RECORDS]; b.last_l2_nodes = c[KCTR_L2_NODES]; b.last_n_k2jobs = c[KCTR_K2JOBS];
    if (b.l2_on && !b.have_counts && getenv("KMDB_VERBOSE"))
        fprintf(stderr, "[kmdb] second level: %u nodes with %u blocks or more joined per tile (indices for %u, entries for %u)\n", c[KCTR_L2_NODES], b.l2_min_blocks,
                b.l2_node_cap, b.l2_ent_cap);
    b.last_records = ((uint64_t)c[KCTR_RECORDS] | ((uint64_t)c[KCTR_RECORDS_HI] << 32)) + (row_mode ? 0u : c[KCTR_WIDE_RECORDS]);
    b.last_n_direct = c[KCTR_DIRECT];
    return 0;
}

}

static void blocks_join_side_streams(kmdb_db* db) {
    if (db->stream2) (void)hipStreamSynchronize(db->stream2);
}

int kmdb_blocks_run(kmdb_db* db, uint32_t* M, uint32_t emit_lo, uint32_t emit_hi, hipStream_t st) {
    BlocksState& b = *db->blocks;
    const uint64_t cells = db->N * (db->N - 1) / 2;
    for (int round = 0; round < 64; ++round) {
        if (b.tile_touched) HIP_TRY(hipMemsetAsync(b.tile_touched, 0, (size_t)b.n_states + 1, st));
        const uint32_t S = std::max<uint32_t>(1u, b.n_slices);
        bool again = false;
        uint64_t records = 0, direct = 0;
        if (b.slice_counts.size() != S) b.slice_counts.assign(S, BlocksState::SliceCounts{});
        bool decoded = false;
        db->last_call_sized = false;
        for (uint32_t k = 0; k < S && !again; ++k) {
            const uint32_t lo = emit_lo + (uint32_t)((uint64_t)(emit_hi - emit_lo) * k / S), hi = emit_lo + (uint32_t)((uint64_t)(emit_hi - emit_lo) * (k + 1) / S);
            if (lo == hi) continue;
            BlocksState::SliceCounts& sc = b.slice_counts[k];
            b.have_counts = sc.valid && sc.lo == lo && sc.hi == hi;
            if (b.have_counts) { b.last_n_wide = sc.n_wide; b.last_n_chunks = sc.n_chunks; b.last_n_raw = sc.n_raw; b.last_n_rowjobs = sc.n_rowjobs; b.last_n_sorted = sc.n_sorted; b.last_n_k2jobs = sc.n_k2jobs; }
            if (!b.have_counts) db->last_call_sized = true;
            bool retry = false;
            if (blocks_attempt(db, M, lo, hi, !decoded, st, &retry)) { blocks_join_side_streams(db); return 1; }
            decoded = true;
            if (!db->fallback_reason.empty()) return 0;
            if (retry) { again = true; for (auto& c : b.slice_counts) c.valid = false; }
            else {
                sc = BlocksState::SliceCounts{true, lo, hi, b.last_n_wide, b.last_n_chunks, b.last_n_raw, b.last_n_rowjobs, b.last_n_sorted, b.last_n_k2jobs};
                records += b.last_records;
                direct += b.last_n_direct;
            }
        }
        if (!again) { b.last_records = records; b.last_n_direct = direct; b.have_counts = true; return 0; }
        HIP_TRY(hipMemsetAsync(M, 0, cells * 4, st));
    }
    return kmdb_set_error("kmdb_blocks_run: the record pools did not converge");
}

kmdb_blocks_counts kmdb_blocks_last_counts(const kmdb_db* db) {
    const BlocksState& b = *db->blocks;
    return kmdb_blocks_counts{b.last_records, b.last_n_direct, b.last_n_wide, b.last_n_chunks, b.l2_on ? b.last_l2_nodes : 0u};
}
const unsigned char* kmdb_blocks_tile_touched(const kmdb_db* db) { return db->blocks ? db->blocks->tile_touched.get() : nullptr; }
```

Measured before the change: 20650 billion.

## Fold per-call memsets into one prologue kernel and drop wide-key pool prefill

```diff
diff --git a/kmer-db_amd/csrc/a2a_blocks.hip b/kmer-db_amd/csrc/a2a_blocks.hip
--- a/kmer-db_amd/csrc/a2a_blocks.hip
+++ b/kmer-db_amd/csrc/a2a_blocks.hip
@@ -203,6 +203,10 @@
         if (v != KEY_NONE && (A.direct || A.t_key[e] != KEY_NONE)) pool_cold(pv)->chunk_fill[v >> CH_SHIFT] = v & (CH_REC - 1u);
     }
 }
+template <class PV> __device__ __forceinline__ void arena_finish_wide(const WaveArena& A, const PV& pv, uint32_t lane) {
+    if (A.dopen && lane < WCH_REC - (A.dslot & (WCH_REC - 1u))) pv.wkey[A.dslot + lane] = KEY_NONE;
+    for (uint32_t k = 0; k < A.wstock; ++k) pv.wkey[(((A.wnext + k) * KMDB_SUBPOOLS + A.wsub) << WCH_SHIFT) + lane] = KEY_NONE;
+}
 
 template <class PV> __device__ __forceinline__ void wide_emit(WaveArena& A, const PV& pv, bool on, unsigned long long rows, unsigned long long cols, uint32_t w, uint32_t stream,
                                           uint32_t lane, unsigned long long lt_mask) {
@@ -316,9 +320,12 @@
     pv.recw[slot] = w;
 }
 
-__global__ void fill_u32_kernel(uint32_t* __restrict__ p, uint32_t n, uint32_t v) {
+__global__ void call_prologue_kernel(uint32_t* __restrict__ state, uint32_t n_state, uint32_t* __restrict__ chunk_fill, uint32_t* __restrict__ chunk_key,
+                                     uint32_t pool_cap, unsigned char* __restrict__ touched, uint32_t n_touched) {
     const uint32_t i = blockIdx.x * blockDim.x + threadIdx.x;
-    if (i < n) p[i] = v;
+    if (i < n_state) state[i] = 0u;
+    if (i < pool_cap) { chunk_fill[i] = 0u; chunk_key[i] = 0xFFFFFFFFu; }
+    if (i < n_touched) touched[i] = 0;
 }
 __global__ void iota_u32_kernel(uint32_t* __restrict__ p, uint32_t n) {
     const uint32_t i = blockIdx.x * blockDim.x + threadIdx.x;
@@ -637,6 +644,8 @@
     ulonglong2* fn_mask;
     uint32_t* fn_blk;
     unsigned long long* widebits;
+    uint32_t* wide_base;
+    uint32_t* wide_slice_cnt;
     uint32_t P, nseg_nodes, n_segs, chain_cap;
     uint32_t emit_lo, emit_hi;
     uint32_t tbits, n_keys;
@@ -754,6 +763,7 @@
     k2_v16i c00 = {}, c10 = {}, c11 = {};
     uint32_t curX = BNONE, n_direct = 0;
     uint32_t flat_n = 0;
+    uint32_t n_flagged = 0;
     auto dflush = [&]() {
         const uint32_t half = lane >> 5, l31 = lane & 31u;
         const uint32_t rb = curX * q.bwidth;
@@ -800,7 +810,8 @@
         const unsigned long long F0 = S.m0, F1 = w1 != BNONE ? S.m1 : 0ull;
         {
             const unsigned long long wb = __ballot(wide);
-            if (lane == 0) q.widebits[base >> 6] = wb;
+            if (lane == 0) { q.widebits[base >> 6] = wb; q.wide_base[base >> 6] = n_flagged; }
+            n_flagged += (uint32_t)__popcll(wb);
         }
         if (__ballot(wide)) {
             const int pl0 = (valid && par >= (int32_t)base) ? (int)(par - (int32_t)base) : (int)lane;
@@ -908,8 +919,10 @@
     KARG(NParams) qe = kernarg_reread<NParams>();
     if (DIRECT && lane == 0 && n_direct) atomicAdd(&qe->direct_ctr[(seg % KMDB_SUBPOOLS) * 16u], n_direct);
     if (FLAT && lane == 0) { qe->slice_cnt[seg] = flat_n; if (flat_n) atomicAdd(&qe->direct_ctr[(seg % KMDB_SUBPOOLS) * 16u], flat_n); }
+    if (lane == 0) qe->wide_slice_cnt[seg] = n_flagged;
     if constexpr (MODE == 0) arena_finish(A, q.pool, lane);
     if constexpr (ROWS) rowtab_finish(RT, pv, lane);
+    else arena_finish_wide(A, pv, lane);
 }
 
 constexpr uint32_t K2D_SLICES = 2;
@@ -1018,23 +1031,74 @@
     }
 }
 
-__global__ void wide_count_kernel(const unsigned long long* __restrict__ bits, uint32_t n_words, uint32_t* __restrict__ cnt) {
+constexpr uint32_t WSL_THREADS = 1024;
+__global__ __launch_bounds__(WSL_THREADS) void wide_slices_kernel(const uint32_t* __restrict__ slice_cnt, uint32_t n_segs, uint32_t* __restrict__ slice_base,
+                                                                   uint32_t* __restrict__ wide_base, uint32_t n_words, uint32_t* __restrict__ counters) {
+    __shared__ uint32_t wtot[WSL_THREADS / WAVE];
+    const uint32_t lane = threadIdx.x & 63u, wave = threadIdx.x >> 6;
+    constexpr uint32_t NW = WSL_THREADS / WAVE;
+    const uint32_t share = ((n_segs + NW - 1u) / NW + 63u) & ~63u;
+    const uint32_t lo = wave * share < n_segs ? wave * share : n_segs;
+    const uint32_t hi = n_segs - lo < share ? n_segs : lo + share;
+    constexpr uint32_t U = 8;
+    uint32_t sum = 0;
+    for (uint32_t i0 = lo; i0 < hi; i0 += U * WAVE) {
+        uint32_t v[U];
+#pragma unroll
+        for (uint32_t j = 0; j < U; ++j) { const uint32_t i = i0 + j * WAVE + lane; v[j] = i < hi ? slice_cnt[i] : 0u; }
+#pragma unroll
+        for (uint32_t j = 0; j < U; ++j) sum += v[j];
+    }
+#pragma unroll
+    for (int d = 32; d >= 1; d >>= 1) sum += (uint32_t)__shfl_xor((int)sum, d, WAVE);
+    if (lane == 0) wtot[wave] = sum;
+    __syncthreads();
+    uint32_t run = 0, total = 0;
+    for (uint32_t k = 0; k < NW; ++k) { const uint32_t t = wtot[k]; if (k < wave) run += t; total += t; }
+    for (uint32_t i0 = lo; i0 < hi; i0 += U * WAVE) {
+        uint32_t v[U];
+#pragma unroll
+        for (uint32_t j = 0; j < U; ++j) { const uint32_t i = i0 + j * WAVE + lane; v[j] = i < hi ? slice_cnt[i] : 0u; }
+#pragma unroll
+        for (uint32_t j = 0; j < U; ++j) {
+            const uint32_t i = i0 + j * WAVE + lane;
+            const uint32_t incl = wave_incl_scan(v[j], lane);
+            if (i < hi) slice_base[i] = run + incl - v[j];
+            run += bcast(incl, WAVE - 1u);
+        }
+    }
+    if (threadIdx.x == 0) { slice_base[n_segs] = total; wide_base[n_words] = total; counters[KCTR_NWIDE] = total; }
+}
+template <bool SERIAL>
+__global__ __launch_bounds__(256) void wide_expand_kernel(const unsigned long long* __restrict__ bits, uint32_t* __restrict__ base, const uint32_t* __restrict__ slice_base,
+                                                          uint32_t words_per_slice, uint32_t slice_shift, uint32_t n_words, uint32_t* __restrict__ widx, uint32_t cap) {
     const uint32_t i = blockIdx.x * blockDim.x + threadIdx.x;
-    if (i < n_words) cnt[i] = (uint32_t)__popcll(bits[i]);
-    else if (i == n_words) cnt[i] = 0;
-}
-__global__ void wide_expand_kernel(const unsigned long long* __restrict__ bits, const uint32_t* __restrict__ base, uint32_t n_words,
-                                   uint32_t* __restrict__ widx, uint32_t cap, uint32_t* __restrict__ counters) {
-    const uint32_t i = blockIdx.x * blockDim.x + threadIdx.x;
-    if (i == 0) counters[KCTR_NWIDE] = base[n_words];
-    if (i >= n_words) return;
-    unsigned long long b = bits[i];
-    uint32_t o = base[i];
-    while (b) {
-        const uint32_t k = (uint32_t)__builtin_ctzll(b);
-        b &= b - 1;
-        if (o < cap) widx[o] = i * 64u + k;
-        ++o;
+    const uint32_t lane = threadIdx.x & 63u;
+    unsigned long long b = 0;
+    uint32_t o = 0;
+    if (i < n_words) {
+        b = bits[i];
+        o = slice_base[slice_shift != 0xFFFFFFFFu ? i >> slice_shift : i / words_per_slice] + base[i];
+        base[i] = o;
+    }
+    if (SERIAL) {
+        while (b) {
+            const uint32_t k = (uint32_t)__builtin_ctzll(b);
+            b &= b - 1;
+            if (o < cap) widx[o] = i * 64u + k;
+            ++o;
+        }
+        return;
+    }
+    const unsigned long long lt_mask = (1ull << lane) - 1ull;
+    unsigned long long todo = __ballot(b != 0ull);
+    const uint32_t w0 = i - lane;
+    while (todo) {
+        const uint32_t j = (uint32_t)__builtin_ctzll(todo);
+        todo &= todo - 1ull;
+        const unsigned long long bj = ((unsigned long long)bcast((uint32_t)(b >> 32), j) << 32) | bcast((uint32_t)b, j);
+        const uint32_t p = bcast(o, j) + (uint32_t)__popcll(bj & lt_mask);
+        if (((bj >> lane) & 1ull) && p < cap) widx[p] = (w0 + j) * 64u + lane;
     }
 }
 
@@ -1491,6 +1555,7 @@
     }
     arena_finish(A, pv, lane);
     if constexpr (ROWS) rowtab_finish(RT, pv, lane);
+    else arena_finish_wide(A, pv, lane);
     if (lane == 0 && n_miss) atomicAdd(&pool_cold(pv)->counters[KCTR_SLOW], n_miss);
     if constexpr (L2) if (lane == 0 && l2_nodes) atomicAdd(&pool_cold(pv)->counters[KCTR_L2_NODES], l2_nodes);
 }
@@ -1899,10 +1964,12 @@
     for (int d = 32; d >= 1; d >>= 1) { mx = max(mx, (uint32_t)__shfl_xor((int)mx, d, WAVE)); nd += (uint32_t)__shfl_xor((int)nd, d, WAVE); }
     if (threadIdx.x == 0) { counters[KCTR_POOL_USED] = mx * KMDB_SUBPOOLS; counters[KCTR_DIRECT] = nd; }
 }
-__global__ void count_raw_kernel(const uint32_t* __restrict__ wsub_cursor, uint32_t* __restrict__ counters) {
+__global__ void count_raw_kernel(const uint32_t* __restrict__ wsub_cursor, uint32_t wsub_cap, uint32_t* __restrict__ counters, uint32_t* __restrict__ handed) {
     uint32_t mx = 0;
-    for (uint32_t p = 0; p < KMDB_SUBPOOLS; ++p) mx = max(mx, wsub_cursor[p * 16u]);
-    counters[KCTR_RAW] = mx * KMDB_SUBPOOLS;
+    for (uint32_t p = threadIdx.x; p < KMDB_SUBPOOLS; p += 64u) { const uint32_t c = wsub_cursor[p * 16u]; mx = max(mx, c); handed[p] = c < wsub_cap ? c : wsub_cap; }
+#pragma unroll
+    for (int d = 32; d >= 1; d >>= 1) mx = max(mx, (uint32_t)__shfl_xor((int)mx, d, WAVE));
+    if (threadIdx.x == 0) counters[KCTR_RAW] = mx * KMDB_SUBPOOLS;
 }
 
 constexpr uint32_t CS_MAX_KEYS = 2048, CS_BLOCKS = 2048, CS_MAX_ROWS = 512;
@@ -1960,18 +2027,33 @@
         row_blk[NB] = blk; row_tab[NB] = tab;
     }
 }
+__device__ __forceinline__ void cs_load_cursors(uint32_t* cur, const uint32_t* __restrict__ wcur) {
+    if (!wcur) return;
+    for (uint32_t k = threadIdx.x; k < KMDB_SUBPOOLS; k += blockDim.x) cur[k] = wcur[k];
+    __syncthreads();
+}
+__device__ __forceinline__ uint32_t cs_chunks_handed(const uint32_t* cur, bool masked, uint32_t t0) {
+    if (!masked) return 0xFFFFFFFFu;
+    const uint32_t c = (t0 >> WCH_SHIFT) + (threadIdx.x & 31u);
+    return (uint32_t)__ballot(c / KMDB_SUBPOOLS < cur[c % KMDB_SUBPOOLS]);
+}
+static_assert(WCH_REC == 64, "cs_chunks_handed: a wave's 64 consecutive slots are one chunk of the wide pool");
 __global__ __launch_bounds__(256) void cs_hist_kernel(const uint32_t* __restrict__ wkey, uint32_t n, uint32_t n_valid, uint32_t n_keys, int mode, const CsRows rows,
-                                                     uint32_t kmask, uint32_t* __restrict__ H) {
+                                                     uint32_t kmask, uint32_t* __restrict__ H, const uint32_t* __restrict__ wcur) {
     extern __shared__ uint32_t cs_lds[];
+    __shared__ uint32_t cs_cur[KMDB_SUBPOOLS];
     const CsJob job = cs_job(mode, n, n_keys, rows);
+    cs_load_cursors(cs_cur, wcur);
     for (uint32_t k = threadIdx.x; k < job.n_bins; k += blockDim.x) cs_lds[k] = 0;
     __syncthreads();
+    const uint32_t wv = threadIdx.x >> 6;
     for (uint32_t i0 = job.lo; i0 < job.hi; i0 += 8u * blockDim.x) {
+        const uint32_t handed = cs_chunks_handed(cs_cur, wcur != nullptr, i0);
         uint32_t kw[8];
 #pragma unroll
         for (uint32_t j = 0; j < 8; ++j) {
             const uint32_t i = i0 + j * blockDim.x + threadIdx.x;
-            kw[j] = i < job.hi ? wkey[i] : 0xFFFFFFFFu;
+            kw[j] = (i < job.hi && ((handed >> (4u * j + wv)) & 1u)) ? wkey[i] : 0xFFFFFFFFu;
         }
 #pragma unroll
         for (uint32_t j = 0; j < 8; ++j) {
@@ -1987,8 +2069,10 @@
 __host__ __device__ inline size_t cs_scatter_lds(uint32_t n_keys, bool packed) { return (size_t)CS_TILE * (sizeof(WideRec) + (packed ? 4 : 8)) + (size_t)n_keys * 12 + CS_THREADS * 4 + 64; }
 __global__ __launch_bounds__(CS_THREADS) void cs_scatter_kernel(const uint32_t* __restrict__ wkey, const WideRec* __restrict__ wrec, uint32_t n, uint32_t n_valid,
                                                          uint32_t n_keys, int mode, const CsRows rows, uint32_t kmask, const uint32_t* __restrict__ O,
-                                                         uint32_t* __restrict__ swkey, WideRec* __restrict__ swrec, uint32_t packed) {
+                                                         uint32_t* __restrict__ swkey, WideRec* __restrict__ swrec, uint32_t packed,
+                                                         const uint32_t* __restrict__ wcur) {
     extern __shared__ __attribute__((aligned(16))) unsigned char cs_raw[];
+    __shared__ uint32_t cs_cur[KMDB_SUBPOOLS];
     WideRec* st_rec = (WideRec*)cs_raw;
     uint32_t* st_dst = (uint32_t*)(st_rec + CS_TILE);
     uint32_t* st_key = st_dst + CS_TILE;
@@ -2003,14 +2087,18 @@
     const uint32_t kper = (nb + CS_THREADS - 1u) / CS_THREADS;
     uint32_t nkw[PER];
     WideRec nrec[PER];
+    const uint32_t wv = threadIdx.x >> 6;
     auto fetch = [&](uint32_t t0) {
+        const uint32_t handed = cs_chunks_handed(cs_cur, wcur != nullptr, t0);
 #pragma unroll
         for (uint32_t j = 0; j < PER; ++j) {
             const uint32_t i = t0 + j * CS_THREADS + threadIdx.x;
             nkw[j] = 0xFFFFFFFFu; nrec[j] = WideRec{0ull, 0ull};
-            if (i < hi) { nkw[j] = wkey[i]; nrec[j] = wrec[i]; }
+            if (i < hi && ((handed >> (4u * j + wv)) & 1u)) { nkw[j] = wkey[i]; nrec[j] = wrec[i]; }
         }
     };
+    static_assert(PER * (CS_THREADS / 64u) == 32u, "cs_chunks_handed covers the 32 chunks of a tile");
+    cs_load_cursors(cs_cur, wcur);
     if (lo < hi) fetch(lo);
     for (uint32_t t0 = lo; t0 < hi; t0 += CS_TILE) {
         for (uint32_t k = threadIdx.x; k < nb; k += CS_THREADS) hist[k] = 0;
@@ -2507,12 +2595,12 @@
     DevBuf<uint16_t> pair_blk;
     DevBuf<unsigned long long> pair_mask;
     uint64_t pair_cap = 0;
-    DevBuf<uint32_t> pair_cursor;
+    uint32_t* pair_cursor = nullptr;
     DevBuf<ulonglong2> fn_mask;
     DevBuf<uint32_t> fn_blk;
     DevBuf<unsigned long long> widebits;
-    DevBuf<uint32_t> wide_cnt;
     DevBuf<uint32_t> wide_base;
+    DevBuf<uint32_t> wide_slice_cnt, wide_slice_base;
     DevBuf<uint32_t> widx;
     DevBuf<uint32_t> wrun_anc;
     DevBuf<uint32_t> wrun_anc_n;
@@ -2527,23 +2615,25 @@
     DevBuf<unsigned char> rec;
     DevBuf<uint32_t> recw;
     uint64_t pool_cap = 0;
-    DevBuf<uint32_t> sub_cursor;
+    uint32_t* sub_cursor = nullptr;
     bool dense_wide = false, dense_narrow = false;
     int k1n_mode = 2;
     DevBuf<unsigned long long> dmask;
     DevBuf<uint32_t> dwx;
     DevBuf<uint32_t> slice_cnt;
-    DevBuf<uint32_t> direct_ctr;
+    uint32_t* direct_ctr = nullptr;
     uint64_t last_n_direct = 0;
     DevBuf<uint32_t> wkey, swkey;
     DevBuf<WideRec> wrec, swrec;
     uint64_t wide_pool_cap = 0;
-    DevBuf<uint32_t> wsub_cursor;
-    DevBuf<uint32_t> run_ctr;
+    uint32_t* wsub_cursor = nullptr;
+    DevBuf<uint32_t> wide_handed;
+    uint32_t* run_ctr = nullptr;
     bool row_mode = false;
     uint32_t rec_pshift = 0;
     uint32_t n_ckeys = 0;
-    DevBuf<uint32_t> ct_hist, ct_offs, ct_cursor;
+    uint32_t* ct_hist = nullptr;
+    DevBuf<uint32_t> ct_offs, ct_cursor;
     DevBuf<void> ct_tmp;
     size_t ct_tmp_bytes = 0;
     DevBuf<uint32_t> rg_hist, rg_offs;
@@ -2562,7 +2652,9 @@
     DevBuf<uint32_t> cs_hist, cs_offs;
     DevBuf<void> cs_tmp;
     size_t cs_tmp_bytes = 0;
-    DevBuf<uint32_t> counters;
+    DevBuf<uint32_t> call_state;
+    uint32_t call_state_n = 0, call_state_n_decode = 0;
+    uint32_t* counters = nullptr;
     uint32_t* h_counters = nullptr;
     bool l2_on = false;
     uint32_t l2_min_blocks = 24, l2_node_cap = 0, l2_ent_cap = 0, last_l2_nodes = 0;
@@ -2579,8 +2671,6 @@
     uint32_t n_slices = 1;
     struct SliceCounts { bool valid = false; uint32_t lo = 0, hi = 0, n_wide = 0, n_chunks = 0, n_raw = 0, n_rowjobs = 0, n_sorted = 0, n_k2jobs = 0; };
     std::vector<SliceCounts> slice_counts;
-    DevBuf<void> scan_tmp;
-    size_t scan_tmp_bytes = 0;
     DevBuf<unsigned char> tile_touched;
     DevBuf<uint32_t> k2j_start;
     DevBuf<uint2> k2j_jobs;
@@ -2789,11 +2879,12 @@
         HIP_TRY(prim::exclusive_sum(nullptr, tb, hist.get(), offs.get(), (int)ne, st));
         DEV_ALLOC(tmp, std::max<size_t>(tb, 16));
         const CsRows no_rows{};
-        hipLaunchKernelGGL(cs_hist_kernel, dim3(CS_BLOCKS_ONE), dim3(256), n_states * 4, st, wkey, nslots, n_states, n_states, (int)CS_BY_STREAM, no_rows, kmask, hist);
+        hipLaunchKernelGGL(cs_hist_kernel, dim3(CS_BLOCKS_ONE), dim3(256), n_states * 4, st, wkey, nslots, n_states, n_states, (int)CS_BY_STREAM, no_rows, kmask, hist,
+                           (const uint32_t*)nullptr);
         HIP_TRY(prim::exclusive_sum(tmp, tb, hist.get(), offs.get(), (int)ne, st));
         HIP_TRY(hipFuncSetAttribute((const void*)cs_scatter_kernel, hipFuncAttributeMaxDynamicSharedMemorySize, (int)cs_scatter_lds(n_states, false)));
         hipLaunchKernelGGL(cs_scatter_kernel, dim3(CS_BLOCKS_ONE), dim3(CS_THREADS), cs_scatter_lds(n_states, false), st, wkey, (const WideRec*)wrec, nslots, n_states, n_states,
-                           (int)CS_BY_STREAM, no_rows, kmask, offs, swkey, swrec, 0u);
+                           (int)CS_BY_STREAM, no_rows, kmask, offs, swkey, swrec, 0u, (const uint32_t*)nullptr);
         total_ptr = offs + (ne - 1);
     } else {
         size_t tb = 0;
@@ -2883,16 +2974,27 @@
     DEV_ALLOC(b.p0_mask, P);
     DEV_ALLOC(b.p0_info, P);
     DEV_ALLOC(b.pair_ofs, P);
-    DEV_ALLOC(b.pair_cursor, (KMDB_PAIR_REGIONS + 1) * 16);
     DEV_ALLOC(b.fn_mask, P);
     DEV_ALLOC(b.fn_blk, P);
     const uint64_t n_words = (P + 63) / 64;
     DEV_ALLOC(b.widebits, n_words);
-    DEV_ALLOC(b.wide_cnt, n_words + 1);
     DEV_ALLOC(b.wide_base, n_words + 1);
-    HIP_TRY(prim::exclusive_sum(nullptr, b.scan_tmp_bytes, b.wide_cnt.get(), b.wide_base.get(), (int)(n_words + 1)));
-    DEV_ALLOC(b.scan_tmp, std::max<size_t>(b.scan_tmp_bytes, 16));
-    DEV_ALLOC(b.counters, KCTR_COUNT);
+    DEV_ALLOC(b.wide_slice_cnt, std::max<size_t>(db->n_nsegs, 1));
+    DEV_ALLOC(b.wide_slice_base, (size_t)db->n_nsegs + 1);
+    DEV_ALLOC(b.wide_handed, KMDB_SUBPOOLS);
+    {
+        uint32_t o = 0;
+        auto take = [&](uint32_t n) { const uint32_t at = o; o += (n + 15u) & ~15u; return at; };
+        const uint32_t o_ctr = take(KCTR_COUNT), o_sub = take(KMDB_SUBPOOLS * 16), o_wsub = take(KMDB_SUBPOOLS * 16), o_run = take(K1W_CTRS * 16),
+                       o_dir = take(KMDB_SUBPOOLS * 16), o_cth = take(b.n_states + 2);
+        b.call_state_n = o;
+        const uint32_t o_pair = take((KMDB_PAIR_REGIONS + 1) * 16);
+        b.call_state_n_decode = o;
+        DEV_ALLOC(b.call_state, o);
+        uint32_t* s = b.call_state;
+        b.counters = s + o_ctr; b.sub_cursor = s + o_sub; b.wsub_cursor = s + o_wsub; b.run_ctr = s + o_run; b.direct_ctr = s + o_dir; b.ct_hist = s + o_cth;
+        b.pair_cursor = s + o_pair;
+    }
     HIP_TRY(hipHostMalloc((void**)&b.h_counters, KCTR_COUNT * 4));
     phase("per-node arrays (hipMalloc)");
     {
@@ -2912,10 +3014,6 @@
         if (alloc_pair_pool(b, std::max<uint64_t>(est_pairs * 2 + P / 4, (uint64_t)KMDB_PAIR_REGIONS * 64))) return 1;
     }
     phase("pair estimate + pair pool");
-    DEV_ALLOC(b.sub_cursor, KMDB_SUBPOOLS * 16);
-    DEV_ALLOC(b.wsub_cursor, KMDB_SUBPOOLS * 16);
-    DEV_ALLOC(b.run_ctr, K1W_CTRS * 16);
-    DEV_ALLOC(b.direct_ctr, KMDB_SUBPOOLS * 16);
     b.dense_wide = true;
     b.dense_narrow = false;
     if (const char* e = getenv("KMDB_DENSE")) b.dense_narrow = atoi(e) >= 2;
@@ -2946,10 +3044,9 @@
         b.key_bits = key_bits;
     }
     DEV_ALLOC(b.tile_touched, (size_t)b.n_states + 1);
-    DEV_ALLOC(b.ct_hist, (size_t)b.n_ckeys + 2);
     DEV_ALLOC(b.ct_offs, (size_t)b.n_ckeys + 2);
     DEV_ALLOC(b.ct_cursor, (size_t)b.n_ckeys + 2);
-    HIP_TRY(prim::exclusive_sum(nullptr, b.ct_tmp_bytes, b.ct_hist.get(), b.ct_offs.get(), (int)(b.n_ckeys + 1), db->stream));
+    HIP_TRY(prim::exclusive_sum(nullptr, b.ct_tmp_bytes, b.ct_hist, b.ct_offs.get(), (int)(b.n_ckeys + 1), db->stream));
     DEV_ALLOC(b.ct_tmp, std::max<size_t>(b.ct_tmp_bytes, 16));
     {
         uint64_t slices = 1;
@@ -2993,7 +3090,8 @@
 uint64_t kmdb_blocks_device_bytes(const kmdb_db* db) {
     if (!db->blocks || !db->blocks->counters) return 0;
     const BlocksState& b = *db->blocks;
-    return db->P * (8 + 4 + 4 + 16 + 4) + (b.dmask ? (uint64_t)db->n_nsegs * db->nseg_nodes * 12 : 0u) + b.pair_cap * 10 + ((b.pool_cap << CH_SHIFT) * 20) + b.pool_cap * 16 + b.wide_cap * 4 + (db->P / 64) * 16 +
+    return db->P * (8 + 4 + 4 + 16 + 4) + (b.dmask ? (uint64_t)db->n_nsegs * db->nseg_nodes * 12 : 0u) + b.pair_cap * 10 + ((b.pool_cap << CH_SHIFT) * 20) + b.pool_cap * 16 + b.wide_cap * 4 + (db->P / 64) * 12 + (uint64_t)db->n_nsegs * 8 +
+           (uint64_t)b.call_state_n_decode * 4 +
            (b.wide_pool_cap << WCH_SHIFT) * (b.row_mode ? 20 : 40) + b.rs_entries * 8 + (uint64_t)b.n_ckeys * 12 +
            (uint64_t)b.NB * (b.l2_node_cap / 64u) * 12 + (uint64_t)b.l2_ent_cap * 26 + (uint64_t)b.l2_node_cap * 4;
 }
@@ -3037,21 +3135,13 @@
     const uint32_t pool_cap = (uint32_t)b.pool_cap;
     const bool row_mode = b.row_mode;
     const uint32_t n_ckeys = b.n_ckeys;
-    HIP_TRY(hipMemsetAsync(b.counters, 0, KCTR_COUNT * 4, st));
-    if (decode) HIP_TRY(hipMemsetAsync(b.pair_cursor, 0, (KMDB_PAIR_REGIONS + 1) * 16 * 4, st));
-    HIP_TRY(hipMemsetAsync(b.sub_cursor, 0, KMDB_SUBPOOLS * 16 * 4, st));
-    HIP_TRY(hipMemsetAsync(b.wsub_cursor, 0, KMDB_SUBPOOLS * 16 * 4, st));
-    HIP_TRY(hipMemsetAsync(b.run_ctr, 0, K1W_CTRS * 16 * 4, st));
-    HIP_TRY(hipMemsetAsync(b.direct_ctr, 0, KMDB_SUBPOOLS * 16 * 4, st));
     auto with_slack = [](uint32_t v) -> uint32_t { return v + v / 8u + 1024u; };
     const uint32_t raw_launch = b.have_counts ? (uint32_t)std::min<uint64_t>(with_slack(b.last_n_raw), row_mode ? 0xFFFFFFFFull : b.wide_pool_cap) : 0u;
-    if (!row_mode) {
-        const uint64_t wslots = b.have_counts ? (uint64_t)raw_launch << WCH_SHIFT : b.wide_pool_cap << WCH_SHIFT;
-        HIP_TRY(hipMemsetAsync(b.wkey, 0xFF, wslots * 4, st));
-    }
-    HIP_TRY(hipMemsetAsync(b.chunk_fill, 0, (size_t)pool_cap * 4, st));
-    HIP_TRY(hipMemsetAsync(b.ct_hist, 0, ((size_t)n_ckeys + 2) * 4, st));
-    hipLaunchKernelGGL(fill_u32_kernel, dim3((pool_cap + 255) / 256), dim3(256), 0, st, b.chunk_key, pool_cap, 0xFFFFFFFFu);
+    {
+        const uint32_t n_state = decode ? b.call_state_n_decode : b.call_state_n, n_touched = decode && b.tile_touched ? b.n_states + 1u : 0u;
+        hipLaunchKernelGGL(call_prologue_kernel, dim3((std::max(std::max(n_state, pool_cap), n_touched) + 255u) / 256u), dim3(256), 0, st, b.call_state.get(), n_state,
+                           b.chunk_fill.get(), b.chunk_key.get(), pool_cap, b.tile_touched.get(), n_touched);
+    }
     if (stage("init")) return 1;
     if (decode) {
         K0Params q{};
@@ -3074,7 +3164,7 @@
         NParams q{};
         q.nl = db->nl; q.parent = db->parent; q.w = db->w; q.dflag = db->dflag; q.seg_anc = db->nseg_anc; q.seg_anc_n = db->nseg_anc_n;
         q.p0_mask = b.p0_mask; q.p0_info = b.p0_info; q.pair_ofs = b.pair_ofs; q.pair_blk = b.pair_blk; q.pair_mask = b.pair_mask;
-        q.fn_mask = b.fn_mask; q.fn_blk = b.fn_blk; q.widebits = b.widebits;
+        q.fn_mask = b.fn_mask; q.fn_blk = b.fn_blk; q.widebits = b.widebits; q.wide_base = b.wide_base; q.wide_slice_cnt = b.wide_slice_cnt;
         q.P = P; q.nseg_nodes = db->nseg_nodes; q.n_segs = db->n_nsegs; q.chain_cap = db->chain_cap;
         q.emit_lo = emit_lo; q.emit_hi = emit_hi; q.tbits = b.dense_narrow ? 0u : arena_table_bits(b.NB); q.n_keys = b.NB;
         q.all_wide = b.dense_narrow ? 1u : 0u;
@@ -3100,7 +3190,7 @@
     auto group_and_apply_chunks = [&](hipStream_t cs) -> int {
         hipLaunchKernelGGL(ct_hist_kernel, dim3((pool_cap + CT_THREADS - 1) / CT_THREADS), dim3(CT_THREADS), 0, cs, b.chunk_key, pool_cap, n_ckeys, b.ct_hist);
         size_t tb = b.ct_tmp_bytes;
-        HIP_TRY(prim::exclusive_sum(b.ct_tmp, tb, b.ct_hist.get(), b.ct_offs.get(), (int)(n_ckeys + 1), cs));
+        HIP_TRY(prim::exclusive_sum(b.ct_tmp, tb, b.ct_hist, b.ct_offs.get(), (int)(n_ckeys + 1), cs));
         HIP_TRY(hipMemcpyAsync(b.ct_cursor, b.ct_offs, ((size_t)n_ckeys + 1) * 4, hipMemcpyDeviceToDevice, cs));
         hipLaunchKernelGGL(ct_scatter_kernel, dim3((pool_cap + CT_THREADS - 1) / CT_THREADS), dim3(CT_THREADS), 0, cs, b.chunk_key, pool_cap, n_ckeys, b.ct_cursor, b.sorted_key, b.sorted_id);
         hipLaunchKernelGGL(ct_count_kernel, dim3(1), dim3(1), 0, cs, b.ct_offs, b.n_states, b.counters);
@@ -3143,12 +3233,12 @@
             if (group_and_apply_chunks(s2)) return 1;
         } else HIP_TRY(hipEventRecord(db->ev_side[1], s2));
     }
-    hipLaunchKernelGGL(wide_count_kernel, dim3((n_words + 1 + 255) / 256), dim3(256), 0, st, b.widebits, n_words, b.wide_cnt);
-    HIP_TRY(prim::exclusive_sum(b.scan_tmp, b.scan_tmp_bytes, b.wide_cnt.get(), b.wide_base.get(), (int)(n_words + 1), st));
+    hipLaunchKernelGGL(wide_slices_kernel, dim3(1), dim3(WSL_THREADS), 0, st, b.wide_slice_cnt.get(), db->n_nsegs, b.wide_slice_base.get(), b.wide_base.get(), n_words,
+                       b.counters);
     uint32_t n_wide;
     if (b.have_counts && b.wide_cap >= b.last_n_wide) n_wide = b.last_n_wide;
     else {
-        HIP_TRY(hipMemcpyAsync(b.h_counters, b.wide_base + n_words, 4, hipMemcpyDeviceToHost, st));
+        HIP_TRY(hipMemcpyAsync(b.h_counters, b.counters + KCTR_NWIDE, 4, hipMemcpyDeviceToHost, st));
         HIP_TRY(hipStreamSynchronize(st));
         n_wide = b.h_counters[0];
         if (n_wide > b.wide_cap) {
@@ -3161,8 +3251,12 @@
         }
     }
     if (!b.widx) { DEV_ALLOC(b.widx, 1); b.wide_cap = std::max<uint64_t>(b.wide_cap, 1); }
-    hipLaunchKernelGGL(wide_expand_kernel, dim3((n_words + 255) / 256), dim3(256), 0, st, b.widebits, b.wide_base, n_words, b.widx,
-                       (uint32_t)b.wide_cap, b.counters);
+    {
+        static const bool wave_form = getenv("KMDB_WIDE_EXPAND") && !strcmp(getenv("KMDB_WIDE_EXPAND"), "wave");
+        const uint32_t wps = db->nseg_nodes / 64u;
+        hipLaunchKernelGGL(wave_form ? wide_expand_kernel<false> : wide_expand_kernel<true>, dim3((n_words + 255) / 256), dim3(256), 0, st, b.widebits.get(), b.wide_base.get(),
+                           b.wide_slice_base.get(), wps, (wps & (wps - 1u)) ? 0xFFFFFFFFu : (uint32_t)__builtin_ctz(wps), n_words, b.widx.get(), (uint32_t)b.wide_cap);
+    }
     if (b.k1n_mode == 2 && !k2d_early && apply_slices()) return 1;
     if (n_wide) {
         WParams q{};
@@ -3274,7 +3368,7 @@
         HIP_TRY(hipGetLastError());
         if (stage("row sort+apply")) return 1;
     } else {
-        hipLaunchKernelGGL(count_raw_kernel, dim3(1), dim3(1), 0, st, b.wsub_cursor, b.counters);
+        hipLaunchKernelGGL(count_raw_kernel, dim3(1), dim3(64), 0, st, b.wsub_cursor, (uint32_t)(b.wide_pool_cap / KMDB_SUBPOOLS), b.counters, b.wide_handed.get());
         uint32_t n_raw;
         if (b.have_counts) n_raw = raw_launch;
         else {
@@ -3287,13 +3381,13 @@
             const CsRows no_rows{};
             const size_t ne = (size_t)b.n_states * CS_BLOCKS_ONE + 1;
             hipLaunchKernelGGL(cs_hist_kernel, dim3(CS_BLOCKS_ONE), dim3(256), b.n_states * 4, st, b.wkey, nslots, b.n_states, b.n_states, (int)CS_BY_STREAM,
-                               no_rows, kmask, b.cs_hist);
+                               no_rows, kmask, b.cs_hist, b.wide_handed.get());
             size_t tb = b.cs_tmp_bytes;
             HIP_TRY(prim::exclusive_sum(b.cs_tmp, tb, b.cs_hist.get(), b.cs_offs.get(), (int)ne, st));
             const bool packed = b.rec_pshift != 0;
             HIP_TRY(hipFuncSetAttribute((const void*)cs_scatter_kernel, hipFuncAttributeMaxDynamicSharedMemorySize, (int)cs_scatter_lds(b.n_states, packed)));
             hipLaunchKernelGGL(cs_scatter_kernel, dim3(CS_BLOCKS_ONE), dim3(CS_THREADS), cs_scatter_lds(b.n_states, packed), st, b.wkey, (const WideRec*)b.wrec, nslots,
-                               b.n_states, b.n_states, (int)CS_BY_STREAM, no_rows, kmask, b.cs_offs, b.swkey, (WideRec*)b.swrec, packed ? 1u : 0u);
+                               b.n_states, b.n_states, (int)CS_BY_STREAM, no_rows, kmask, b.cs_offs, b.swkey, (WideRec*)b.swrec, packed ? 1u : 0u, b.wide_handed.get());
             const uint32_t* total_ptr = b.cs_offs + (ne - 1);
             HIP_TRY(hipMemcpyAsync(b.counters + KCTR_WIDE_RECORDS, total_ptr, 4, hipMemcpyDeviceToDevice, st));
             if (getenv("KMDB_K2_WINDOWS") && !packed) {
@@ -3419,7 +3513,6 @@
     BlocksState& b = *db->blocks;
     const uint64_t cells = db->N * (db->N - 1) / 2;
     for (int round = 0; round < 64; ++round) {
-        if (b.tile_touched) HIP_TRY(hipMemsetAsync(b.tile_touched, 0, (size_t)b.n_states + 1, st));
         const uint32_t S = std::max<uint32_t>(1u, b.n_slices);
         bool again = false;
         uint64_t records = 0, direct = 0;
```

New measurement: 21100 billion, median of 6. +2.2%, better.
